# sikang/motion_primitive_library

Measured on NVIDIA H100. Metric: node-expansions/sec (frontier x |U| primitives validated+costed) on 512^3 voxel map, higher is better.
Workload: dtype f64

## Files before the change

### motion_primitive_library_b200/csrc/mplx_api.cu

```cuda
#include <cuda_runtime.h>
#include <math.h>
#include <stdarg.h>
#include <stdio.h>
#include <stdlib.h>
#include <string.h>

#include <new>
#include <vector>

#include "../../include/mplx.h"
#include "mplx_internal.h"
#include "mplx_pack.cuh"

namespace mplx {
thread_local char g_err[512] = "";
int fail(int code, const char *fmt, ...) {
  va_list ap;
  va_start(ap, fmt);
  vsnprintf(g_err, sizeof g_err, fmt, ap);
  va_end(ap);
  return code;
}
}
using mplx::g_err;

int mplx_bind(mplx_ctx *ctx) {
  if (!ctx) return fail(MPLX_ERR_ARG, "null ctx");
  CU(cudaSetDevice(ctx->device));
  return MPLX_OK;
}

static void refresh_params(mplx_ctx *c) {
  c->P.map = c->has_map ? c->map.p : nullptr;
  c->P.pot = c->has_pot ? c->pot.p : nullptr;
  c->P.region_bits = c->has_region ? c->region.p : nullptr;
  c->P.U = c->U.p;
  c->P.stats = c->stats_on ? c->stats.p : nullptr;
  c->P.occ_bits = c->has_map ? c->occ.p : nullptr;
  c->P.occ2 = c->has_map ? c->occ2.p : nullptr;
  c->P.occ2_bytes = c->has_map ? c->occ2_window : 0;
  c->P.prow = c->prow.p;
  c->P.row_u = c->row_u.p;
  c->P.row_axis = c->row_axis.p;
  c->P.n_rows = c->n_rows;
  c->P.ttab = c->ttab.p;
  c->P.tcount = c->tcount.p;
  c->P.tdt = c->tdt.p;
  int maxn = mplx::kNMax;
  if (c->has_map && c->has_params && (c->P.control & 15) != MPLX_VEL && c->P.v_max > 0) {
    const double nb = ceil(c->P.v_max * c->P.T / c->P.res);
    if (nb < (double)mplx::kNMax) maxn = nb < 5 ? 5 : (int)nb;
  }
  c->P.maxn = maxn;
}

extern "C" {

const char *mplx_last_error(void) { return g_err; }

const char *mplx_build_info(void) {
  return "libmplx sm_90a; nvcc -gencode arch=compute_90a,code=sm_90a -fmad=false; "
         "IEEE double, no CPU fallback";
}

int mplx_create(int dim, int device, mplx_ctx **out) {
  if (!out) return fail(MPLX_ERR_ARG, "out is null");
  *out = nullptr;
  if (dim != 2 && dim != 3) return fail(MPLX_ERR_ARG, "dim must be 2 or 3, got %d", dim);
  int ndev = 0;
  cudaError_t e = cudaGetDeviceCount(&ndev);
  if (e != cudaSuccess || ndev == 0) {
    cudaGetLastError();
    return fail(MPLX_ERR_CUDA, "no CUDA device available (%s); libmplx has no CPU fallback",
                e == cudaSuccess ? "device count is 0" : cudaGetErrorString(e));
  }
  if (device < 0 || device >= ndev) return fail(MPLX_ERR_ARG, "device %d out of range [0,%d)", device, ndev);
  CU(cudaSetDevice(device));
  mplx_ctx *c = new (std::nothrow) mplx_ctx();
  if (!c) return fail(MPLX_ERR_ALLOC, "host allocation failed");
  c->dim = dim;
  c->device = device;
  if (const char *k = getenv("MPLX_KERNEL")) {
    const int w = atoi(k);
    if (w >= 0 && w <= 5) c->kernel = w;
  }
  memset(&c->P, 0, sizeof c->P);
  c->P.dim = dim;
  e = cudaStreamCreateWithFlags(&c->stream, cudaStreamNonBlocking);
  if (e != cudaSuccess) {
    delete c;
    return fail(MPLX_ERR_CUDA, "cudaStreamCreate failed: %s", cudaGetErrorString(e));
  }
  e = c->stats.reserve(2);
  if (e != cudaSuccess) {
    cudaStreamDestroy(c->stream);
    delete c;
    return fail(MPLX_ERR_ALLOC, "cudaMalloc failed: %s", cudaGetErrorString(e));
  }
  *out = c;
  return MPLX_OK;
}

int mplx_destroy(mplx_ctx *c) {
  if (!c) return MPLX_OK;
  cudaSetDevice(c->device);
  cudaStreamSynchronize(c->stream);
  c->map.release(); c->pot.release(); c->region.release(); c->U.release(); c->stats.release();
  c->prow.release(); c->row_axis.release(); c->row_u.release();
  c->occ.release(); c->occ2.release(); c->ttab.release(); c->tcount.release(); c->tdt.release();
  for (int b = 0; b < kPackBufs; b++) c->cb[b].release();
  if (c->d2h_stream) cudaStreamDestroy(c->d2h_stream);
  c->eb.release(); c->fxq.release(); c->ub.release(); c->sb.release(); c->tun.release(); c->tb.release();
  c->d_nodes.release(); c->d_succ.release(); c->d_count.release(); c->d_action.release();
  c->d_lattice.release(); c->d_cost.release(); c->d_key.release();
  c->h_nodes.release(); c->h_succ.release(); c->h_count.release(); c->h_action.release();
  c->h_lattice.release(); c->h_cost.release(); c->h_key.release();
  cudaStreamDestroy(c->stream);
  delete c;
  return MPLX_OK;
}

int mplx_set_map(mplx_ctx *c, const int8_t *data, const int32_t *dim, const double *origin, double res) {
  if (int r = mplx_bind(c)) return r;
  if (!data || !dim || !origin) return fail(MPLX_ERR_ARG, "null argument");
  if (!(res > 0)) return fail(MPLX_ERR_ARG, "res must be > 0");
  size_t nvox = 1;
  for (int k = 0; k < c->dim; k++) {
    if (dim[k] <= 0) return fail(MPLX_ERR_ARG, "dim[%d] = %d", k, dim[k]);
    nvox *= (size_t)dim[k];
  }
  if (nvox >= (size_t)1 << 31) return fail(MPLX_ERR_ARG, "grid has %zu cells; getIndex is int32 (map_util.h:34-41)", nvox);
  CU(cudaStreamSynchronize(c->stream));
  CU(c->map.reserve(nvox));
  CU(cudaMemcpyAsync(c->map.p, data, nvox, cudaMemcpyHostToDevice, c->stream));
  CU(c->occ.reserve((nvox + 31) / 32));
  CU(mplx::launch_pack_bits(c->map.p, nvox, c->occ.p, true, c->stream));
  const int nz = c->dim == 3 ? dim[2] : 1;
  const size_t npairs = mplx::occ2_pair_count(c->dim, dim[0], dim[1], nz);
  CU(c->occ2.reserve(2 * npairs));
  CU(mplx::launch_pack_occ2(c->occ.p, nvox, c->dim, dim[0], dim[1], nz, c->occ2.p, c->stream));
  c->launches += 2;
  {
    int maxp = 0, maxw = 0;
    cudaDeviceGetAttribute(&maxp, cudaDevAttrMaxPersistingL2CacheSize, c->device);
    cudaDeviceGetAttribute(&maxw, cudaDevAttrMaxAccessPolicyWindowSize, c->device);
    const size_t half = npairs * sizeof(uint32_t);
    const size_t bytes = 2 * half <= (size_t)maxp ? 2 * half : half;
    c->occ2_window = 0;
    if (maxp > 0 && maxw > 0) {
      const size_t want = bytes < (size_t)maxp ? bytes : (size_t)maxp;
      if (cudaDeviceSetLimit(cudaLimitPersistingL2CacheSize, want) == cudaSuccess)
        c->occ2_window = bytes < (size_t)maxw ? bytes : (size_t)maxw;
      else
        cudaGetLastError();
    }
  }
  CU(cudaStreamSynchronize(c->stream));
  c->nvox = nvox;
  for (int k = 0; k < 3; k++) {
    c->P.mdim[k] = k < c->dim ? dim[k] : 1;
    c->P.origin[k] = k < c->dim ? origin[k] : 0.0;
    c->P.dimd[k] = (double)c->P.mdim[k];
  }
  c->P.occ2_nb[0] = mplx::occ2_bricks_x(c->dim, dim[0]);
  c->P.occ2_nb[1] = mplx::occ2_bricks_y(c->dim, dim[1]);
  c->P.occ2_sum = (unsigned)npairs;
  c->P.res = res;
  c->P.rinv = 1.0 / res;
  c->has_map = true;
  c->has_pot = false;
  c->has_region = false;
  c->tun.release();
  refresh_params(c);
  return MPLX_OK;
}

int mplx_set_potential(mplx_ctx *c, const int8_t *data, double pw, double gw) {
  if (int r = mplx_bind(c)) return r;
  if (!c->has_map) return fail(MPLX_ERR_ARG, "mplx_set_map must be called first");
  c->P.pot_w = pw;
  c->P.grad_w = gw;
  if (!data) {
    c->has_pot = false;
  } else {
    CU(cudaStreamSynchronize(c->stream));
    CU(c->pot.reserve(c->nvox));
    CU(cudaMemcpyAsync(c->pot.p, data, c->nvox, cudaMemcpyHostToDevice, c->stream));
    CU(cudaStreamSynchronize(c->stream));
    c->has_pot = true;
  }
  refresh_params(c);
  return MPLX_OK;
}

int mplx_set_potential_weights(mplx_ctx *c, double pw, double gw) {
  if (int r = mplx_bind(c)) return r;
  c->P.pot_w = pw;
  c->P.grad_w = gw;
  return MPLX_OK;
}

int mplx_set_search_region(mplx_ctx *c, const uint8_t *in_region) {
  if (int r = mplx_bind(c)) return r;
  if (!c->has_map) return fail(MPLX_ERR_ARG, "mplx_set_map must be called first");
  if (!in_region) {
    c->has_region = false;
  } else {
    CU(cudaStreamSynchronize(c->stream));
    DevBuf<uint8_t> tmp;
    CU(tmp.reserve(c->nvox));
    cudaError_t e = cudaMemcpyAsync(tmp.p, in_region, c->nvox, cudaMemcpyHostToDevice, c->stream);
    if (e == cudaSuccess) e = c->region.reserve((c->nvox + 31) / 32);
    if (e == cudaSuccess) e = mplx::launch_pack_bits((const int8_t *)tmp.p, c->nvox, c->region.p, false, c->stream);
    if (e == cudaSuccess) e = cudaStreamSynchronize(c->stream);
    tmp.release();
    CU(e);
    c->launches++;
    c->has_region = true;
  }
  refresh_params(c);
  return MPLX_OK;
}

int mplx_set_params(mplx_ctx *c, int control, double T, double w, double wyaw, double v_max,
                    double a_max, double j_max, double yaw_max, const double *U, int nU, int udim) {
  if (int r = mplx_bind(c)) return r;
  const int base = control & 15;
  if ((control & ~31) || (base != MPLX_VEL && base != MPLX_ACC && base != MPLX_JRK && base != MPLX_SNP))
    return fail(MPLX_ERR_ARG, "control 0x%x is not a Control::Control value (control.h:10-20)", control);
  const bool yaw = control & 16;
  if (!U || nU <= 0 || nU > mplx::kMaxU) return fail(MPLX_ERR_ARG, "need 1 <= nU <= %d controls", mplx::kMaxU);
  if (udim != c->dim + (yaw ? 1 : 0))
    return fail(MPLX_ERR_ARG, "udim %d must be dim%s = %d for control 0x%x", udim, yaw ? "+1" : "", c->dim + (yaw ? 1 : 0), control);
  if (!(T > 0)) return fail(MPLX_ERR_ARG, "T (dt_) must be > 0");
  CU(cudaStreamSynchronize(c->stream));
  CU(c->U.reserve((size_t)nU * udim));
  CU(cudaMemcpyAsync(c->U.p, U, sizeof(double) * nU * udim, cudaMemcpyHostToDevice, c->stream));
  {
    std::vector<unsigned char> prow((size_t)nU * 3, 0), row_axis;
    std::vector<double> row_u;
    bool fits = true;
    for (int a = 0; a < c->dim && fits; a++) {
      const size_t first = row_u.size();
      for (int i = 0; i < nU; i++) {
        const double v = U[(size_t)i * udim + a];
        size_t r = first;
        for (; r < row_u.size(); r++)
          if (memcmp(&row_u[r], &v, sizeof v) == 0) break;
        if (r == row_u.size()) {
          if (row_u.size() >= 255) { fits = false; break; }
          row_u.push_back(v);
          row_axis.push_back((unsigned char)a);
        }
        prow[(size_t)i * 3 + a] = (unsigned char)r;
      }
    }
    c->n_rows = 0;
    if (fits) {
      CU(c->prow.reserve(prow.size()));
      CU(c->row_u.reserve(row_u.size()));
      CU(c->row_axis.reserve(row_axis.size()));
      CU(cudaMemcpyAsync(c->prow.p, prow.data(), prow.size(), cudaMemcpyHostToDevice, c->stream));
      CU(cudaMemcpyAsync(c->row_u.p, row_u.data(), sizeof(double) * row_u.size(), cudaMemcpyHostToDevice, c->stream));
      CU(cudaMemcpyAsync(c->row_axis.p, row_axis.data(), row_axis.size(), cudaMemcpyHostToDevice, c->stream));
      CU(cudaStreamSynchronize(c->stream));
      c->n_rows = (int)row_u.size();
    }
  }
  CU(c->ttab.reserve((size_t)(mplx::kNMax + 1) * mplx::kTStride + 8));
  CU(c->tcount.reserve(mplx::kNMax + 1));
  CU(c->tdt.reserve(mplx::kNMax + 1));
  CU(cudaMemsetAsync(c->ttab.p, 0, sizeof(double) * ((size_t)(mplx::kNMax + 1) * mplx::kTStride + 8), c->stream));
  CU(mplx::launch_build_ttab(T, c->ttab.p, c->tcount.p, c->tdt.p, c->stream));
  c->launches++;
  CU(cudaStreamSynchronize(c->stream));
  c->P.control = control;
  c->P.nU = nU;
  c->P.udim = udim;
  c->P.T = T;
  c->P.w = w;
  c->P.wyaw = wyaw;
  c->P.v_max = v_max;
  c->P.a_max = a_max;
  c->P.j_max = j_max;
  c->P.yaw_max = yaw_max;
  c->P.cos_yaw_max = cos(yaw_max);
  c->has_params = true;
  refresh_params(c);
  return MPLX_OK;
}

int mplx_check_ready(mplx_ctx *c, int n_nodes) {
  if (!c->has_map) return fail(MPLX_ERR_ARG, "no map: call mplx_set_map first");
  if (!c->has_params) return fail(MPLX_ERR_ARG, "no params: call mplx_set_params first");
  if (n_nodes < 0) return fail(MPLX_ERR_ARG, "n_nodes < 0");
  if ((size_t)n_nodes * c->P.nU >= ((size_t)1 << 31)) return fail(MPLX_ERR_ARG, "batch too large");
  return MPLX_OK;
}
static int check_ready(mplx_ctx *c, int n_nodes, const mplx_succ_out *out) {
  if (int r = mplx_check_ready(c, n_nodes)) return r;
  if (!out || !out->count) return fail(MPLX_ERR_ARG, "out->count is required");
  return MPLX_OK;
}

int mplx_expand_device(mplx_ctx *c, const void *d_nodes, int n_nodes, const mplx_succ_out *out, void *stream) {
  if (int r = mplx_bind(c)) return r;
  if (int r = check_ready(c, n_nodes, out)) return r;
  if (n_nodes == 0) return MPLX_OK;
  if (!d_nodes) return fail(MPLX_ERR_ARG, "d_nodes is null");
  cudaStream_t st = stream ? (cudaStream_t)stream : c->stream;
  if (c->stats_on) CU(cudaMemsetAsync(c->stats.p, 0, 2 * sizeof(unsigned long long), st));
  CU(c->fxq.reserve((size_t)n_nodes * c->P.nU));
  int launches = 0;
  CU(mplx::launch_expand(c->P, (const mplx_waypoint *)d_nodes, n_nodes, *out, st, c->kernel, &c->fxq.view, &launches));
  c->launches += launches;
  if (c->stats_on)
    CU(cudaMemcpyAsync(c->last_stats, c->stats.p, 2 * sizeof(unsigned long long), cudaMemcpyDeviceToHost, st));
  return MPLX_OK;
}

int mplx_expand(mplx_ctx *c, const mplx_waypoint *nodes, int n_nodes, const mplx_succ_out *out) {
  if (int r = mplx_bind(c)) return r;
  if (int r = check_ready(c, n_nodes, out)) return r;
  if (n_nodes == 0) return MPLX_OK;
  if (!nodes) return fail(MPLX_ERR_ARG, "nodes is null");
  const int nU = c->P.nU;
  int chunk = (1 << 20) / nU;
  if (chunk < 1) chunk = 1;
  if (chunk > n_nodes) chunk = n_nodes;
  const size_t slots = (size_t)chunk * nU;
  cudaStream_t st = c->stream;

  CU(c->d_nodes.reserve(chunk));
  CU(c->d_count.reserve(chunk));
  if (out->succ) CU(c->d_succ.reserve(slots));
  if (out->cost) CU(c->d_cost.reserve(slots));
  if (out->action) CU(c->d_action.reserve(slots));
  if (out->key) CU(c->d_key.reserve(slots));
  if (out->lattice) CU(c->d_lattice.reserve(slots * MPLX_LATTICE_MAX));

  const bool pin_nodes = is_pinned(nodes), pin_count = is_pinned(out->count), pin_succ = is_pinned(out->succ),
             pin_cost = is_pinned(out->cost), pin_action = is_pinned(out->action), pin_key = is_pinned(out->key),
             pin_lat = is_pinned(out->lattice);
  if (!pin_nodes) CU(c->h_nodes.reserve(chunk));
  if (!pin_count) CU(c->h_count.reserve(chunk));
  if (out->succ && !pin_succ) CU(c->h_succ.reserve(slots));
  if (out->cost && !pin_cost) CU(c->h_cost.reserve(slots));
  if (out->action && !pin_action) CU(c->h_action.reserve(slots));
  if (out->key && !pin_key) CU(c->h_key.reserve(slots));
  if (out->lattice && !pin_lat) CU(c->h_lattice.reserve(slots * MPLX_LATTICE_MAX));

  static const bool no_zero_copy = getenv("MPLX_NO_ZERO_COPY") != nullptr;
  if (!no_zero_copy && !c->stats_on && (size_t)n_nodes * nU <= 4096) {
    const int m = n_nodes;
    const size_t sm = (size_t)m * nU;
    const mplx_waypoint *src = nodes;
    if (!pin_nodes) {
      memcpy(c->h_nodes.p, nodes, sizeof(mplx_waypoint) * m);
      src = c->h_nodes.p;
    }
    mplx_succ_out d;
    d.count = pin_count ? out->count : c->h_count.p;
    d.succ = out->succ ? (pin_succ ? out->succ : c->h_succ.p) : nullptr;
    d.cost = out->cost ? (pin_cost ? out->cost : c->h_cost.p) : nullptr;
    d.action = out->action ? (pin_action ? out->action : c->h_action.p) : nullptr;
    d.key = out->key ? (pin_key ? out->key : c->h_key.p) : nullptr;
    d.lattice = out->lattice ? (pin_lat ? out->lattice : c->h_lattice.p) : nullptr;
    CU(c->fxq.reserve(sm));
    int launches = 0;
    CU(mplx::launch_expand(c->P, src, m, d, st, c->kernel, &c->fxq.view, &launches));
    c->launches += launches;
    CU(cudaStreamSynchronize(st));
    if (!pin_count) memcpy(out->count, c->h_count.p, sizeof(int32_t) * m);
    if (out->succ && !pin_succ) memcpy(out->succ, c->h_succ.p, sizeof(mplx_waypoint) * sm);
    if (out->cost && !pin_cost) memcpy(out->cost, c->h_cost.p, sizeof(double) * sm);
    if (out->action && !pin_action) memcpy(out->action, c->h_action.p, sizeof(int32_t) * sm);
    if (out->key && !pin_key) memcpy(out->key, c->h_key.p, sizeof(uint64_t) * sm);
    if (out->lattice && !pin_lat) memcpy(out->lattice, c->h_lattice.p, sizeof(int32_t) * sm * MPLX_LATTICE_MAX);
    return MPLX_OK;
  }

  unsigned long long acc_stats[2] = {0, 0};
  for (int off = 0; off < n_nodes; off += chunk) {
    const int m = n_nodes - off < chunk ? n_nodes - off : chunk;
    const size_t so = (size_t)off * nU, sm = (size_t)m * nU;
    const mplx_waypoint *src = nodes + off;
    if (!pin_nodes) {
      memcpy(c->h_nodes.p, src, sizeof(mplx_waypoint) * m);
      src = c->h_nodes.p;
    }
    CU(cudaMemcpyAsync(c->d_nodes.p, src, sizeof(mplx_waypoint) * m, cudaMemcpyHostToDevice, st));
    mplx_succ_out d;
    d.count = c->d_count.p;
    d.succ = out->succ ? c->d_succ.p : nullptr;
    d.cost = out->cost ? c->d_cost.p : nullptr;
    d.action = out->action ? c->d_action.p : nullptr;
    d.key = out->key ? c->d_key.p : nullptr;
    d.lattice = out->lattice ? c->d_lattice.p : nullptr;
    if (c->stats_on) CU(cudaMemsetAsync(c->stats.p, 0, 2 * sizeof(unsigned long long), st));
    CU(c->fxq.reserve((size_t)m * nU));
    int launches = 0;
    CU(mplx::launch_expand(c->P, c->d_nodes.p, m, d, st, c->kernel, &c->fxq.view, &launches));
    c->launches += launches;
    if (c->stats_on)
      CU(cudaMemcpyAsync(c->last_stats, c->stats.p, 2 * sizeof(unsigned long long), cudaMemcpyDeviceToHost, st));
#define D2H(field, T, mult, pinflag, hbuf)                                                              \
  if (out->field) {                                                                                    \
    T *dst = pinflag ? out->field + so * (mult) : hbuf.p;                                              \
    CU(cudaMemcpyAsync(dst, d.field, sizeof(T) * sm * (mult), cudaMemcpyDeviceToHost, st));             \
  }
    {
      int32_t *dst = pin_count ? out->count + off : c->h_count.p;
      CU(cudaMemcpyAsync(dst, d.count, sizeof(int32_t) * m, cudaMemcpyDeviceToHost, st));
    }
    D2H(succ, mplx_waypoint, 1, pin_succ, c->h_succ)
    D2H(cost, double, 1, pin_cost, c->h_cost)
    D2H(action, int32_t, 1, pin_action, c->h_action)
    D2H(key, uint64_t, 1, pin_key, c->h_key)
    D2H(lattice, int32_t, MPLX_LATTICE_MAX, pin_lat, c->h_lattice)
#undef D2H
    CU(cudaStreamSynchronize(st));
    if (!pin_count) memcpy(out->count + off, c->h_count.p, sizeof(int32_t) * m);
    if (out->succ && !pin_succ) memcpy(out->succ + so, c->h_succ.p, sizeof(mplx_waypoint) * sm);
    if (out->cost && !pin_cost) memcpy(out->cost + so, c->h_cost.p, sizeof(double) * sm);
    if (out->action && !pin_action) memcpy(out->action + so, c->h_action.p, sizeof(int32_t) * sm);
    if (out->key && !pin_key) memcpy(out->key + so, c->h_key.p, sizeof(uint64_t) * sm);
    if (out->lattice && !pin_lat)
      memcpy(out->lattice + so * MPLX_LATTICE_MAX, c->h_lattice.p, sizeof(int32_t) * sm * MPLX_LATTICE_MAX);
    if (c->stats_on) {
      acc_stats[0] += c->last_stats[0];
      acc_stats[1] += c->last_stats[1];
    }
  }
  if (c->stats_on) {
    c->last_stats[0] = acc_stats[0];
    c->last_stats[1] = acc_stats[1];
  }
  return MPLX_OK;
}

int mplx_set_kernel(mplx_ctx *c, int which) {
  if (!c) return fail(MPLX_ERR_ARG, "null ctx");
  if (which < 0 || which > 5)
    return fail(MPLX_ERR_ARG, "which must be 0 (auto), 1 (sequential), 2 (register), 3 (flat), 4 (dealing) or 5 (fixed-point)");
  c->kernel = which;
  return MPLX_OK;
}

int mplx_sync(mplx_ctx *c) {
  if (int r = mplx_bind(c)) return r;
  CU(cudaStreamSynchronize(c->stream));
  return MPLX_OK;
}

int64_t mplx_launch_count(const mplx_ctx *c) { return c ? c->launches : 0; }

int mplx_enable_stats(mplx_ctx *c, int on) {
  if (int r = mplx_bind(c)) return r;
  c->stats_on = on != 0;
  refresh_params(c);
  return MPLX_OK;
}

int mplx_last_stats(mplx_ctx *c, int64_t *samples, int64_t *successors) {
  if (int r = mplx_bind(c)) return r;
  CU(cudaStreamSynchronize(c->stream));
  if (samples) *samples = (int64_t)c->last_stats[0];
  if (successors) *successors = (int64_t)c->last_stats[1];
  return MPLX_OK;
}

void *mplx_stream(mplx_ctx *c) { return c ? (void *)c->stream : nullptr; }

void *mplx_host_alloc(size_t bytes) {
  void *p = nullptr;
  if (cudaHostAlloc(&p, bytes, cudaHostAllocDefault) != cudaSuccess) {
    cudaGetLastError();
    fail(MPLX_ERR_ALLOC, "cudaHostAlloc(%zu) failed", bytes);
    return nullptr;
  }
  return p;
}

void mplx_host_free(void *p) {
  if (p) cudaFreeHost(p);
}

}
```

### motion_primitive_library_b200/csrc/mplx_device.cuh

```cuda
#pragma once
#include <limits.h>
#include <stdint.h>

namespace mplx {

struct EnvParams {
  int dim, control, nU, udim;
  double T, w, wyaw;
  double v_max, a_max, j_max, yaw_max;
  double cos_yaw_max;
  int mdim[3];
  double origin[3];
  double res;
  double rinv;
  double dimd[3];
  double pot_w, grad_w;
  const int8_t *map;
  const int8_t *pot;
  const uint32_t *region_bits;
  const double *U;
  unsigned long long *stats;
  const uint32_t *occ_bits;
  const double *ttab;
  const int *tcount;
  const double *tdt;
  int maxn;
  const uint32_t *occ2;
  unsigned occ2_sum;
  size_t occ2_bytes;
  int occ2_nb[2];
  const unsigned char *prow;
  const double *row_u;
  const unsigned char *row_axis;
  int n_rows;
};

constexpr int kNMax = 128;
constexpr int kTStride = kNMax + 2;

#define MPLX_PI 3.14159265358979323846

__device__ __forceinline__ double normalize_angle(double a) {
  while (a > MPLX_PI) a -= 2.0 * MPLX_PI;
  while (a < -MPLX_PI) a += 2.0 * MPLX_PI;
  return a;
}

__device__ __forceinline__ uint64_t hash_premix(int v) {
  uint64_t k = (uint64_t)(int64_t)v;
  const uint64_t m = 0xc6a4a7935bd1e995ULL;
  k *= m;
  k ^= k >> 47;
  k *= m;
  return k;
}
__device__ __forceinline__ void hash_fold(uint64_t &h, uint64_t k) {
  const uint64_t m = 0xc6a4a7935bd1e995ULL;
  h ^= k;
  h *= m;
  h += 0xe6546b64ULL;
}
__device__ __forceinline__ void hash_combine(uint64_t &h, int v) { hash_fold(h, hash_premix(v)); }

#define MPLX_MAGIC 6755399441055744.0

__device__ __forceinline__ double div_exact(double a, double b, double binv) {
  const double q0 = a * binv;
  const double r = __fma_rn(-b, q0, a);
  return __fma_rn(r, binv, q0);
}

__device__ __forceinline__ double round_haz(double x, int &k) {
  const double m = x + MPLX_MAGIC;
  double kd = m - MPLX_MAGIC;
  const double f = x - kd;
  k = __double2loint(m);
  if (fabs(f) == 0.5) {
    if (f > 0.0 && x > 0.0) { kd += 1.0; k += 1; }
    if (f < 0.0 && x < 0.0) { kd -= 1.0; k -= 1; }
  }
  return kd;
}

__device__ __forceinline__ int float_to_int(double p, double origin, double res) {
  const double x = (p - origin) / res - 0.5;
  if (!(fabs(x) < 2147483648.0)) return INT_MIN;
  int k;
  round_haz(x, k);
  return k;
}

__device__ __forceinline__ int lattice_id(double x, double res, double rinv) {
  int k;
  round_haz(div_exact(x, res, rinv), k);
  return k;
}

__device__ __forceinline__ double ceil_exact(double x) {
  const double kd = (x + MPLX_MAGIC) - MPLX_MAGIC;
  return kd < x ? kd + 1.0 : kd;
}

template <int ORD>
struct Axis {
  double c1, c2, c3, c4, c5;

  __device__ __forceinline__ void build(double u, double p, double v, double a, double j) {
    c1 = c2 = c3 = 0.0;
    if (ORD == 1) { c4 = u; c5 = p; }
    if (ORD == 2) { c3 = u; c4 = v; c5 = p; }
    if (ORD == 3) { c2 = u; c3 = a; c4 = v; c5 = p; }
    if (ORD == 4) { c1 = u; c2 = j; c3 = a; c4 = v; c5 = p; }
  }

  template <bool EXACT_ZERO>
  __device__ __forceinline__ double p(double t, double pw3, double pw4) const {
    if (EXACT_ZERO) {
      double s = 0.0;
      if (ORD >= 4) s = s + c1 / 24 * pw4;
      if (ORD >= 3) s = s + c2 / 6 * pw3;
      if (ORD >= 2) s = s + c3 / 2 * t * t;
      s = s + c4 * t;
      return s + c5;
    }
    if (ORD == 1) return c4 * t + c5;
    if (ORD == 2) return c3 / 2 * t * t + c4 * t + c5;
    if (ORD == 3) return c2 / 6 * pw3 + c3 / 2 * t * t + c4 * t + c5;
    return c1 / 24 * pw4 + c2 / 6 * pw3 + c3 / 2 * t * t + c4 * t + c5;
  }
  __device__ __forceinline__ double v(double t, double pw3) const {
    double s = 0.0;
    if (ORD >= 4) s = s + c1 / 6 * pw3;
    if (ORD >= 3) s = s + c2 / 2 * t * t;
    if (ORD >= 2) s = s + c3 * t;
    return s + c4;
  }
  __device__ __forceinline__ double a(double t) const {
    double s = 0.0;
    if (ORD >= 4) s = s + c1 / 2 * t * t;
    if (ORD >= 3) s = s + c2 * t;
    return s + c3;
  }
  __device__ __forceinline__ double j(double t) const {
    double s = 0.0;
    if (ORD >= 4) s = s + c1 * t;
    return s + c2;
  }

  __device__ __forceinline__ double max_vel(double T) const {
    double pw3T = (T * T) * T;
    double m = fmax(fabs(v(0.0, 0.0)), fabs(v(T, pw3T)));
    if (ORD >= 4 && c1 / 2 != 0) {
      double b = c1 / 2, c = c2, d = c3;
      double disc = c * c - 4 * b * d;
      if (!(disc < 0)) {
        double r0 = (-c - sqrt(disc)) / (2 * b);
        double r1 = (-c + sqrt(disc)) / (2 * b);
        bool brk = false;
        if (r0 > 0 && r0 < T) {
          double vv = fabs(v(r0, (r0 * r0) * r0));
          m = vv > m ? vv : m;
        } else if (r0 >= T)
          brk = true;
        if (!brk && r1 > 0 && r1 < T) {
          double vv = fabs(v(r1, (r1 * r1) * r1));
          m = vv > m ? vv : m;
        }
      }
    } else if (ORD >= 3 && c2 != 0) {
      double r = -c3 / c2;
      if (r > 0 && r < T) {
        double vv = fabs(v(r, (r * r) * r));
        m = vv > m ? vv : m;
      }
    }
    return m;
  }
  __device__ __forceinline__ double max_acc(double T) const {
    double m = fmax(fabs(a(0.0)), fabs(a(T)));
    if (ORD >= 4 && c1 != 0) {
      double r = -c2 / c1;
      if (r > 0 && r < T) {
        double aa = fabs(a(r));
        m = aa > m ? aa : m;
      }
    }
    return m;
  }
  __device__ __forceinline__ double max_jrk(double T) const { return fmax(fabs(j(0.0)), fabs(j(T))); }

  __device__ __forceinline__ double J(double T) const {
    double u = ORD == 1 ? c4 : ORD == 2 ? c3 : ORD == 3 ? c2 : c1;
    return u * u * T;
  }
};

__device__ __forceinline__ double dot2_normalized(double v0, double v1, double c, double s) {
  double z = v0 * v0 + v1 * v1;
  double n0 = v0, n1 = v1;
  if (z > 0) {
    double nn = sqrt(z);
    n0 = v0 / nn;
    n1 = v1 / nn;
  }
  return n0 * c + n1 * s;
}

}
```

### motion_primitive_library_b200/csrc/mplx_fx.cu

```cuda
#include "mplx_dispatch.h"
#include "mplx_fx.cuh"
#include "mplx_pack.cuh"

namespace mplx {

constexpr int kFxThreads = kThreads + 32;

struct FxShared {
  unsigned long long amask[kThreads];
  uint64_t hcurr[kThreads];
  double intrinsic[kThreads];
  unsigned slot[kThreads];
  uint32_t vbits[9];
  int q_n;
  unsigned char q[kThreads];
  unsigned char n[kThreads];
  unsigned char full[kThreads];
};

template <int DIM, int ORD, bool REGION>
__device__ __forceinline__ void fx_resolve(const EnvParams &P, const mplx_waypoint *__restrict__ nodes, int node0,
                                           int nU, int inv_nU, const FxShared &S, int lane, double *__restrict__ cost) {
  const int qn = S.q_n;
  for (int i = lane; i < qn; i += 32) {
    const int owner = S.q[i];
    const int nl = (owner * inv_nU) >> 20;
    const int ci = owner - nl * nU;
    const mplx_waypoint *cp = nodes + node0 + nl;
    const double *u = P.U + (size_t)ci * P.udim;
    PrimState<DIM, ORD, false> q;
#pragma unroll
    for (int k = 0; k < DIM; k++) q.ax[k].build(__ldg(u + k), cp->pos[k], cp->vel[k], cp->acc[k], cp->jrk[k]);
    double cf[CoefLayout<DIM, ORD, false>::NCMAX];
    fill_coef<DIM, ORD, false>(q, false, cf);
    const int n = S.n[owner];
    const double *tt = P.ttab + (size_t)n * kTStride;
    unsigned long long m = S.amask[owner];
    const int count = __ldg(P.tcount + n);
    const bool full = S.full[owner] != 0;
    bool blocked = false;
    for (int k = 0; !blocked; k++) {
      if (full) {
        if (k >= count) break;
      } else {
        if (m == 0) break;
        k = __ffsll((long long)m) - 1;
        m &= m - 1;
      }
      double pk[DIM];
      eval_pos<DIM, ORD>(cf, __ldg(tt + k), pk);
      int idx;
      blocked = !sample_cell<DIM>(P, pk, idx);
      if (!blocked) {
        blocked = (__ldg(P.occ_bits + (idx >> 5)) >> (idx & 31)) & 1u;
        if (REGION) blocked = blocked || !((__ldg(P.region_bits + (idx >> 5)) >> (idx & 31)) & 1u);
      }
    }
    if (cost) cost[S.slot[owner]] = blocked ? (double)INFINITY : 0.0 + S.intrinsic[owner];
  }
}

template <int DIM, int ORD, int UNR, int MINB, bool LAT, bool REGION>
__global__ void __launch_bounds__(kFxThreads, MINB)
expand_fx_kernel(const __grid_constant__ EnvParams P, const mplx_waypoint *__restrict__ nodes, int n_nodes, int npb,
                 int inv_nU, const __grid_constant__ OutPtrs o) {
  __shared__ FxShared S;
  const int nU = P.nU;
  const int items = npb * nU;
  const int node0 = blockIdx.x * npb;
  if (threadIdx.x >= kThreads) {
    const int lane = threadIdx.x - kThreads;
    if (lane == 0) S.q_n = 0;
    for (int j = lane; j < npb; j += 32)
      if (node0 + j < n_nodes) S.hcurr[j] = curr_hash<DIM, ORD>(nodes + node0 + j);
    __syncthreads();
    __syncthreads();
    __syncthreads();
    fx_resolve<DIM, ORD, REGION>(P, nodes, node0, nU, inv_nU, S, lane, o.cost);
    return;
  }

  const int item = threadIdx.x;
  const int nl = (item * inv_nU) >> 20;
  const int ci = item - nl * nU;
  const int ni = node0 + nl;
  const bool active = item < items && ni < n_nodes;
  PrimState<DIM, ORD, false> pr;
  bool ok = false, same = true;
  double max_v = 0;
  mplx_waypoint tn;
  int lat[LAT ? MPLX_LATTICE_MAX : 1];
  uint64_t key = 0;
  if (active) {
    const mplx_waypoint *cp = nodes + ni;
    const double *u = P.U + (size_t)ci * P.udim;
#pragma unroll
    for (int k = 0; k < DIM; k++) pr.ax[k].build(__ldg(u + k), cp->pos[k], cp->vel[k], cp->acc[k], cp->jrk[k]);
    const double T = P.T;
    const double pw3T = (T * T) * T, pw4T = pw3T * T;
#pragma unroll
    for (int k = 0; k < 3; k++) {
      if (k < DIM) {
        tn.pos[k] = pr.ax[k].template p<true>(T, pw3T, pw4T);
        tn.vel[k] = pr.ax[k].v(T, pw3T);
        tn.acc[k] = pr.ax[k].a(T);
        tn.jrk[k] = pr.ax[k].j(T);
        same = same && (pr.ax[k].c5 == tn.pos[k]);
      } else {
        tn.pos[k] = tn.vel[k] = tn.acc[k] = tn.jrk[k] = 0.0;
      }
    }
    tn.yaw = 0.0;
    tn.t = cp->t + T;
    ok = true;
#pragma unroll
    for (int k = 0; k < DIM; k++) {
      const double mv = pr.ax[k].max_vel(T);
      if (ORD >= 2 && P.v_max > 0) ok = ok && !(mv > P.v_max);
      if (mv > max_v) max_v = mv;
    }
    if (ok && ORD >= 3 && P.a_max > 0) {
#pragma unroll
      for (int k = 0; k < DIM; k++) ok = ok && !(pr.ax[k].max_acc(T) > P.a_max);
    }
    if (ok && ORD >= 4 && P.j_max > 0) {
#pragma unroll
      for (int k = 0; k < DIM; k++) ok = ok && !(pr.ax[k].max_jrk(T) > P.j_max);
    }
    if (ok) {
      int nl_ = 0;
#pragma unroll
      for (int k = 0; k < DIM; k++) {
        int id = lattice_id(tn.pos[k], 0.01, 100.0);
        hash_combine(key, id);
        if (LAT) lat[nl_++] = id;
        if (ORD >= 2) { id = lattice_id(tn.vel[k], 0.1, 10.0); hash_combine(key, id); if (LAT) lat[nl_++] = id; }
        if (ORD >= 3) { id = lattice_id(tn.acc[k], 0.1, 10.0); hash_combine(key, id); if (LAT) lat[nl_++] = id; }
        if (ORD >= 4) { id = lattice_id(tn.jrk[k], 0.1, 10.0); hash_combine(key, id); if (LAT) lat[nl_++] = id; }
      }
      if (LAT) {
#pragma unroll
        for (int q = 0; q < MPLX_LATTICE_MAX; q++)
          if (q >= nl_) lat[q] = 0;
      }
    }
  }
  __syncthreads();
  const bool emit = ok && key != S.hcurr[nl];

  const unsigned bal = __ballot_sync(0xffffffffu, emit);
  if ((threadIdx.x & 31) == 0) S.vbits[item >> 5] = bal;
  __syncthreads();
  size_t slot = 0;
  if (active) {
    const int s = nl * nU;
    int rank = 0;
    for (int wd = s >> 5; wd <= (item >> 5); wd++) {
      uint32_t m = S.vbits[wd];
      const int lo = wd << 5;
      if (s > lo) m &= ~0u << (s - lo);
      if (item < lo + 32) m &= (1u << (item - lo)) - 1u;
      rank += __popc(m);
    }
    if (ci == nU - 1) o.count[ni] = rank + (emit ? 1 : 0);
    if (emit) {
      slot = (size_t)ni * nU + rank;
      if (o.succ) store_waypoint(o.succ + slot, tn);
      if (o.action) __stcs(o.action + slot, ci);
      if (o.key) __stcs(reinterpret_cast<unsigned long long *>(o.key + slot), (unsigned long long)key);
      if (LAT && o.lattice) {
#pragma unroll
        for (int q = 0; q < MPLX_LATTICE_MAX; q++) o.lattice[slot * MPLX_LATTICE_MAX + q] = lat[q];
      }
    }
  }

  if (emit) {
    int verdict = 0;
    const double intrinsic = intrinsic_cost<DIM, ORD, false>(P, pr);
    if (!same) {
      double dt;
      const int n = sample_count_n(P, max_v, dt);
      double reach = 0.0;
#pragma unroll
      for (int a = 0; a < DIM; a++) reach = fmax(reach, (fabs(pr.ax[a].c5) + fabs(P.origin[a])) * P.rinv);
      if (n > kNMax || !(reach < kFxRange)) {
        double cf[CoefLayout<DIM, ORD, false>::NCMAX];
        fill_coef<DIM, ORD, false>(pr, false, cf);
        unsigned ns = 0;
        verdict = isinf(traverse_loop<DIM, ORD, false>(P, cf, false, max_v, ns)) ? 1 : 0;
      } else {
        double C[DIM][ORD + 1];
#pragma unroll
        for (int a = 0; a < DIM; a++) fx_axis<ORD>(pr.ax[a], P.origin[a], P.rinv, C[a]);
        const unsigned *__restrict__ occ_words = P.occ2;
        unsigned long long amask = 0;
        bool full = false;
        double t = 0;
        int base = 0;
        for (int left = __ldg(P.tcount + n);; left -= UNR, base += UNR) {
          unsigned amb;
          const int st = fx_group<DIM, ORD, UNR, REGION>(P, occ_words, C, dt, left, t, amb);
          if (st == 2) {
            verdict = 1;
            break;
          }
          if (amb) {
            if (base + UNR <= 64)
              amask |= (unsigned long long)amb << base;
            else
              full = true;
          }
          if (st == 1) break;
        }
        if (verdict == 0 && (amask != 0 || full)) {
          verdict = 2;
          const int qi = atomicAdd(&S.q_n, 1);
          S.q[qi] = (unsigned char)threadIdx.x;
          S.amask[threadIdx.x] = amask;
          S.n[threadIdx.x] = (unsigned char)n;
          S.full[threadIdx.x] = full ? 1 : 0;
          S.slot[threadIdx.x] = (unsigned)slot;
          S.intrinsic[threadIdx.x] = intrinsic;
        }
      }
    }
    if (verdict != 2 && o.cost) o.cost[slot] = verdict == 1 ? (double)INFINITY : 0.0 + intrinsic;
  }
  __syncthreads();
}

bool fx_supported(const EnvParams &P) {
  return P.occ2 != nullptr && P.pot == nullptr && (P.control & 16) == 0 && P.nU <= kThreads && P.stats == nullptr;
}

cudaError_t launch_expand_fx(const EnvParams &P, const mplx_waypoint *d_nodes, int n_nodes, const OutPtrs &o,
                             cudaStream_t st) {
  static const int unr_env = [] {
    const char *e = getenv("MPLX_FX_UNR");
    return e ? atoi(e) : 0;
  }();
  static const int minb_env = [] {
    const char *e = getenv("MPLX_FX_MINB");
    return e ? atoi(e) : 0;
  }();
  const int unr = unr_env == 4 || unr_env == 8 ? unr_env : (P.maxn <= 15 ? 4 : 8);
  const int npb = kThreads / P.nU;
  const int grid = (n_nodes + npb - 1) / npb;
  const int inv_nU = ((1 << 20) + P.nU - 1) / P.nU;
  return with_dim(P.dim, [&](auto DIM) {
    return with_order(P.control, [&](auto ORD) {
      return with_bool(unr == 8, [&](auto UNR8) {
        return with_bool(o.lattice != nullptr, [&](auto LAT) {
          return with_bool(P.region_bits != nullptr, [&](auto REGION) {
            auto launch = [&](auto MINB) {
              expand_fx_kernel<DIM, ORD, UNR8 ? 8 : 4, MINB, LAT, REGION>
                  <<<grid, kFxThreads, 0, st>>>(P, d_nodes, n_nodes, npb, inv_nU, o);
              return cudaGetLastError();
            };
            if constexpr (DIM == 3 && ORD == 2 && !LAT && !REGION) {
              if (minb_env == 5) return launch(Int<5>());
              if (minb_env == 6) return launch(Int<6>());
            }
            return launch(Int<4>());
          });
        });
      });
    });
  });
}

__global__ void pack_occ2_kernel(const uint32_t *__restrict__ occ, size_t nvox, int dim, int nx, int ny, int nz,
                                 uint32_t *__restrict__ out) {
  const size_t npairs = occ2_pair_count(dim, nx, ny, nz);
  for (size_t p = (size_t)blockIdx.x * blockDim.x + threadIdx.x; p < npairs; p += (size_t)gridDim.x * blockDim.x) {
    uint32_t o, s;
    occ2_brick_pair(occ, p, nvox, dim, nx, ny, nz, o, s);
    out[p] = o;
    out[npairs + p] = s;
  }
}

cudaError_t launch_pack_occ2(const uint32_t *d_occ, size_t nvox, int dim, int nx, int ny, int nz, uint32_t *d_out,
                             cudaStream_t st) {
  const size_t npairs = occ2_pair_count(dim, nx, ny, nz);
  int grid = (int)((npairs + 255) / 256);
  if (grid > sm_count() * 16) grid = sm_count() * 16;
  if (grid < 1) grid = 1;
  pack_occ2_kernel<<<grid, 256, 0, st>>>(d_occ, nvox, dim, nx, ny, nz, d_out);
  return cudaGetLastError();
}

}
```

### motion_primitive_library_b200/csrc/mplx_fx.cuh

```cuda
#pragma once
#include "mplx_expand.cuh"
#include "mplx_pack.cuh"

namespace mplx {

constexpr double kFxMagic = 1572864.0;
constexpr int kFxHiBase = 0x41380000;
constexpr double kFxEps = 0x1p-26;
constexpr unsigned kFxUnc = 128u;
constexpr double kFxRange = 131072.0;

template <int ORD>
__device__ __forceinline__ void fx_axis(const Axis<ORD> &ax, double origin, double rinv, double (&C)[ORD + 1]) {
  double q[5];
  q[0] = ax.c5;
  q[1] = ax.c4;
  q[2] = ax.c3 / 2;
  q[3] = ax.c2 / 6;
  q[4] = ax.c1 / 24;
#pragma unroll
  for (int i = 1; i <= ORD; i++) C[i] = q[i] * rinv;
  C[0] = (q[0] - origin) * rinv + (kFxMagic + kFxEps);
}

__device__ __forceinline__ unsigned rotr_wrap(unsigned x, unsigned s) {
  unsigned r;
  asm("shf.r.wrap.b32 %0, %1, %1, %2;" : "=r"(r) : "r"(x), "r"(s));
  return r;
}

template <int DIM, int ORD, int UNR, bool REGION>
__device__ __forceinline__ int fx_group(const EnvParams &P, const unsigned *__restrict__ base,
                                        const double (&C)[DIM][ORD + 1], double dt, int left, double &t, unsigned &amb) {
  unsigned w[UNR], rot[UNR];
  unsigned uncm = 0;
#pragma unroll
  for (int j = 0; j < UNR; j++) {
    int cell[DIM];
    unsigned lo[DIM];
    bool inside = true;
#pragma unroll
    for (int a = 0; a < DIM; a++) {
      double h = C[a][ORD];
#pragma unroll
      for (int i = ORD - 1; i >= 1; i--) h = __fma_rn(h, t, C[a][i]);
      const double m = __fma_rn(h, t, C[a][0]);
      cell[a] = __double2hiint(m) - kFxHiBase;
      lo[a] = (unsigned)__double2loint(m);
      inside = inside && ((unsigned)cell[a] < (unsigned)P.mdim[a]);
    }
    const unsigned fr = DIM == 3 ? min(min(lo[0], lo[1]), lo[DIM - 1]) : min(lo[0], lo[1]);
    const unsigned ub = fr < kFxUnc ? 1u : 0u;
    uncm += ub << j;
    w[j] = 0xffffffffu;
    if (REGION) {
      int idx = cell[0] + P.mdim[0] * cell[1];
      if (DIM == 3) idx += P.mdim[0] * P.mdim[1] * cell[DIM - 1];
      rot[j] = (unsigned)(idx - j);
      if (inside && !ub) {
        const unsigned wi = (unsigned)idx >> 5;
        w[j] = __ldg(P.occ_bits + wi) | ~__ldg(P.region_bits + wi);
      }
    } else {
      const int z = DIM == 3 ? cell[DIM - 1] : 0;
      rot[j] = occ2_bit<DIM>(cell[0], cell[1]) - j;
      if (inside) w[j] = __ldg(base + (occ2_pair<DIM>(cell[0], cell[1], z, P.occ2_nb[0], P.occ2_nb[1]) + (ub ? P.occ2_sum : 0u)));
    }
    t += dt;
  }
  unsigned r = 0;
#pragma unroll
  for (int j = 0; j < UNR; j++) r |= rotr_wrap(w[j], rot[j]) & (1u << j);
  if (left < UNR) r &= (1u << left) - 1u;
  amb = r & uncm;
  if (r & ~uncm) return 2;
  return left <= UNR ? 1 : 0;
}

template <int UNR>
struct FxWords {
  unsigned w[UNR], rot[UNR];
  unsigned uncm;
};

template <int DIM, int ORD, int UNR, bool REGION>
__device__ __forceinline__ void fx_issue(const EnvParams &P, const unsigned *__restrict__ base,
                                         const double (&C)[DIM][ORD + 1], double dt, double &t, FxWords<UNR> &G) {
  G.uncm = 0;
#pragma unroll
  for (int j = 0; j < UNR; j++) {
    int cell[DIM];
    unsigned lo[DIM];
    bool inside = true;
#pragma unroll
    for (int a = 0; a < DIM; a++) {
      double h = C[a][ORD];
#pragma unroll
      for (int i = ORD - 1; i >= 1; i--) h = __fma_rn(h, t, C[a][i]);
      const double m = __fma_rn(h, t, C[a][0]);
      cell[a] = __double2hiint(m) - kFxHiBase;
      lo[a] = (unsigned)__double2loint(m);
      inside = inside && ((unsigned)cell[a] < (unsigned)P.mdim[a]);
    }
    const unsigned fr = DIM == 3 ? min(min(lo[0], lo[1]), lo[DIM - 1]) : min(lo[0], lo[1]);
    const unsigned ub = fr < kFxUnc ? 1u : 0u;
    G.uncm += ub << j;
    G.w[j] = 0xffffffffu;
    if (REGION) {
      int idx = cell[0] + P.mdim[0] * cell[1];
      if (DIM == 3) idx += P.mdim[0] * P.mdim[1] * cell[DIM - 1];
      G.rot[j] = (unsigned)(idx - j);
      if (inside && !ub) {
        const unsigned wi = (unsigned)idx >> 5;
        G.w[j] = __ldg(P.occ_bits + wi) | ~__ldg(P.region_bits + wi);
      }
    } else {
      const int z = DIM == 3 ? cell[DIM - 1] : 0;
      G.rot[j] = occ2_bit<DIM>(cell[0], cell[1]) - j;
      if (inside) G.w[j] = __ldg(base + (occ2_pair<DIM>(cell[0], cell[1], z, P.occ2_nb[0], P.occ2_nb[1]) + (ub ? P.occ2_sum : 0u)));
    }
    t += dt;
  }
}

template <int UNR>
__device__ __forceinline__ int fx_decide(const FxWords<UNR> &G, int left, unsigned &amb) {
  unsigned r = 0;
#pragma unroll
  for (int j = 0; j < UNR; j++) r |= rotr_wrap(G.w[j], G.rot[j]) & (1u << j);
  if (left < UNR) r &= (1u << left) - 1u;
  amb = r & G.uncm;
  if (r & ~G.uncm) return 2;
  return left <= UNR ? 1 : 0;
}

template <int DIM, int ORD, int UNR, bool REGION>
__device__ __forceinline__ int fx_traverse(const EnvParams &P, const double (&C)[DIM][ORD + 1], double dt, int count,
                                           unsigned long long &amask, bool &full) {
  const unsigned *__restrict__ base = P.occ2;
  amask = 0;
  full = false;
  double t = 0;
  int left = count, k0 = 0;
  FxWords<UNR> A, B;
  fx_issue<DIM, ORD, UNR, REGION>(P, base, C, dt, t, A);
  for (;;) {
    unsigned amb;
    int st;
    if (left > UNR) fx_issue<DIM, ORD, UNR, REGION>(P, base, C, dt, t, B);
    st = fx_decide<UNR>(A, left, amb);
    if (st == 2) return 1;
    if (amb) {
      if (k0 + UNR <= 64) amask |= (unsigned long long)amb << k0; else full = true;
    }
    if (st == 1) return 0;
    left -= UNR;
    k0 += UNR;
    if (left > UNR) fx_issue<DIM, ORD, UNR, REGION>(P, base, C, dt, t, A);
    st = fx_decide<UNR>(B, left, amb);
    if (st == 2) return 1;
    if (amb) {
      if (k0 + UNR <= 64) amask |= (unsigned long long)amb << k0; else full = true;
    }
    if (st == 1) return 0;
    left -= UNR;
    k0 += UNR;
  }
}

template <int DIM, int ORD>
__device__ __forceinline__ uint64_t curr_hash(const mplx_waypoint *cp) {
  uint64_t h = 0;
#pragma unroll
  for (int k = 0; k < DIM; k++) {
    hash_combine(h, lattice_id(cp->pos[k], 0.01, 100.0));
    if (ORD >= 2) hash_combine(h, lattice_id(cp->vel[k], 0.1, 10.0));
    if (ORD >= 3) hash_combine(h, lattice_id(cp->acc[k], 0.1, 10.0));
    if (ORD >= 4) hash_combine(h, lattice_id(cp->jrk[k], 0.1, 10.0));
  }
  return h;
}

constexpr unsigned kFxSegments = 64;

struct FxAmbRec {
  unsigned slot;
  int node;
  unsigned short action;
  unsigned char n;
  unsigned char full;
  unsigned long long amask;
};

}
```

### motion_primitive_library_b200/csrc/mplx_fxn.cu

```cuda
#include <string.h>

#include "mplx_dispatch.h"
#include "mplx_fx.cuh"
#include "mplx_span.cuh"

namespace mplx {

template <int ORD>
struct FxnRow {
  double st[4];
  double C[ORD + 1];
  double mv;
  double J;
  int id[4];
  uint64_t km[ORD];
  unsigned char f0, f1, f2, pad[5];
};
constexpr unsigned char kSame = 1, kReach = 2, kVel = 1, kAcc = 1, kJrk = 2;


struct FxnWork {
  unsigned rows_n;
  unsigned slot;
};

constexpr int kMaxNpb = kThreads / 9;
struct FxnShared {
  uint64_t hcurr[kMaxNpb];
  uint64_t ckm[kMaxNpb * 3 * 4];
  double tcurr[kMaxNpb];
  FxnWork work[kThreads];
  unsigned char owner[kThreads];
  uint32_t vbits[8];
  unsigned short cnt[kWarps][33], start[kWarps][33];
};
constexpr unsigned kNoWork = 0xffffffffu;

struct FxnStage {
  int succ, key, action, cost;
};
constexpr int kSpanUnsorted = 7, kSpanMinLoop = 20;

__device__ __forceinline__ void bulk_copy(void *g, const unsigned char *s, unsigned bytes) {
  const unsigned sa = (unsigned)__cvta_generic_to_shared(s);
  asm volatile("cp.async.bulk.global.shared::cta.bulk_group [%0], [%1], %2;" ::"l"(g), "r"(sa), "r"(bytes) : "memory");
}

__device__ __forceinline__ void span_out(void *g, const unsigned char *s, unsigned elem, unsigned n) {
  const SpanCopy c = span_copy(reinterpret_cast<uintptr_t>(g), elem, n);
  unsigned char *d = static_cast<unsigned char *>(g);
  const unsigned end = elem * n, trail0 = end - c.trail;
  for (unsigned i = 0; i < c.lead; i += 4) *reinterpret_cast<uint32_t *>(d + i) = *reinterpret_cast<const uint32_t *>(s + i);
  for (unsigned i = trail0; i < end; i += 4) *reinterpret_cast<uint32_t *>(d + i) = *reinterpret_cast<const uint32_t *>(s + i);
  unsigned at = c.lead;
  if (c.head) bulk_copy(d + at, s + at, c.head);
  at += c.head;
  if (c.body) bulk_copy(d + at, s + at, c.body);
  at += c.body;
  if (c.tail) bulk_copy(d + at, s + at, c.tail);
}

template <int DIM, int ORD, int UNR, int MINB, bool LAT, bool REGION, bool SORT, bool STAGE>
__global__ void __launch_bounds__(kThreads, MINB)
expand_fxn_kernel(const __grid_constant__ EnvParams P, const mplx_waypoint *__restrict__ nodes, int n_nodes, int npb,
                  int inv_nU, int inv_rows, FxAmbRec *__restrict__ amb_q, unsigned *__restrict__ amb_n,
                  unsigned amb_cap, const __grid_constant__ OutPtrs o, int pf_ahead, const FxnStage sg) {
  extern __shared__ __align__(16) unsigned char fx_dyn[];
  FxnRow<ORD> *rows = reinterpret_cast<FxnRow<ORD> *>(fx_dyn);
  __shared__ FxnShared S;
  const int nU = P.nU;
  const int items = npb * nU;
  const int node0 = blockIdx.x * npb;
  const int n_rows = P.n_rows;
  const int lane = threadIdx.x & 31, warp = threadIdx.x >> 5;

  if (SORT) {
    for (int b = threadIdx.x; b < kWarps * 33; b += kThreads) (&S.cnt[0][0])[b] = 0;
    S.work[threadIdx.x].slot = kNoWork;
  }
  if (pf_ahead > 0 && threadIdx.x < 16) {
    const long long first = ((long long)blockIdx.x + pf_ahead) * npb;
    const char *pfp = reinterpret_cast<const char *>(nodes + first) + 128 * threadIdx.x;
    if (first < n_nodes && pfp < reinterpret_cast<const char *>(nodes + min((long long)n_nodes, first + npb)))
      asm volatile("prefetch.global.L2 [%0];" ::"l"(pfp));
  }

  {
    const double T = P.T;
    const int R = npb * n_rows;
    const int tail = (3 * R) & (kThreads - 1);
    const bool hash_warp = warp == (tail <= kThreads - 32 ? kWarps - 1 : tail >> 5);
    double cx[2] = {0.0, 0.0}, ct = 0.0;
    auto load_ids = [&] {
      constexpr int F = DIM * ORD;
#pragma unroll
      for (int k = 0; k < 2; k++) {
        const int q = lane + 32 * k;
        const int j = q / F, af = q - j * F;
        if (q < npb * F && node0 + j < n_nodes)
          cx[k] = reinterpret_cast<const double *>(nodes + node0 + j)[(af % ORD) * 3 + af / ORD];
      }
      if (lane < npb && node0 + lane < n_nodes) ct = nodes[node0 + lane].t;
    };
    if (hash_warp) load_ids();
    for (int it = threadIdx.x; it < 3 * R; it += kThreads) {
      const int part = it >= 2 * R ? 2 : (it >= R ? 1 : 0);
      const int r = it - part * R;
      const int nl = (r * inv_rows) >> 20;
      const int rr = r - nl * n_rows;
      if (node0 + nl >= n_nodes) continue;
      const mplx_waypoint *cp = nodes + node0 + nl;
      const int a = __ldg(P.row_axis + rr);
      Axis<ORD> ax;
      ax.build(__ldg(P.row_u + rr), cp->pos[a], cp->vel[a], cp->acc[a], cp->jrk[a]);
      FxnRow<ORD> &Rw = rows[r];
      if (part == 0) {
        const double origin = a == 0 ? P.origin[0] : (a == 1 ? P.origin[1] : P.origin[2]);
        const double pw3T = (T * T) * T, pw4T = pw3T * T;
        const double pos = ax.template p<true>(T, pw3T, pw4T);
        Rw.st[0] = pos;
        const int id = lattice_id(pos, 0.01, 100.0);
        Rw.id[0] = id;
        Rw.km[0] = hash_premix(id);
        unsigned char f = 0;
        if (ax.c5 == pos) f |= kSame;
        if ((fabs(ax.c5) + fabs(origin)) * P.rinv < kFxRange) f |= kReach;
        Rw.f0 = f;
        Rw.J = ax.J(T);
      } else if (part == 1) {
        const double pw3T = (T * T) * T;
        const double vel = ax.v(T, pw3T);
        Rw.st[1] = vel;
        const int id = ORD >= 2 ? lattice_id(vel, 0.1, 10.0) : 0;
        Rw.id[1] = id;
        if (ORD >= 2) Rw.km[ORD >= 2 ? 1 : 0] = hash_premix(id);
        const double mv = ax.max_vel(T);
        Rw.mv = mv;
        Rw.f1 = (ORD >= 2 && P.v_max > 0 && mv > P.v_max) ? 0 : kVel;
      } else {
        const double origin = a == 0 ? P.origin[0] : (a == 1 ? P.origin[1] : P.origin[2]);
        fx_axis<ORD>(ax, origin, P.rinv, Rw.C);
        const double acc = ax.a(T), jrk = ax.j(T);
        Rw.st[2] = acc;
        Rw.st[3] = jrk;
        Rw.id[2] = ORD >= 3 ? lattice_id(acc, 0.1, 10.0) : 0;
        Rw.id[3] = ORD >= 4 ? lattice_id(jrk, 0.1, 10.0) : 0;
        if (ORD >= 3) Rw.km[ORD >= 3 ? 2 : 0] = hash_premix(Rw.id[2]);
        if (ORD >= 4) Rw.km[ORD >= 4 ? 3 : 0] = hash_premix(Rw.id[3]);
        unsigned char f = kAcc | kJrk;
        if (ORD >= 3 && P.a_max > 0 && ax.max_acc(T) > P.a_max) f &= ~kAcc;
        if (ORD >= 4 && P.j_max > 0 && ax.max_jrk(T) > P.j_max) f &= ~kJrk;
        Rw.f2 = f;
      }
    }
    if (hash_warp) {
      constexpr int F = DIM * ORD;
#pragma unroll
      for (int k = 0; k < 2; k++) {
        const int q = lane + 32 * k;
        if (q < npb * F) {
          const bool is_pos = (q % F) % ORD == 0;
          S.ckm[q] = hash_premix(lattice_id(cx[k], is_pos ? 0.01 : 0.1, is_pos ? 100.0 : 10.0));
        }
      }
      for (int q = lane + 64; q < npb * F; q += 32) {
        const int j = q / F, af = q - j * F;
        const bool is_pos = af % ORD == 0;
        const double x = node0 + j < n_nodes ? reinterpret_cast<const double *>(nodes + node0 + j)[(af % ORD) * 3 + af / ORD] : 0.0;
        S.ckm[q] = hash_premix(lattice_id(x, is_pos ? 0.01 : 0.1, is_pos ? 100.0 : 10.0));
      }
      __syncwarp();
      for (int j = lane; j < npb; j += 32) {
        uint64_t h = 0;
#pragma unroll
        for (int af = 0; af < F; af++) hash_fold(h, S.ckm[j * F + af]);
        S.hcurr[j] = h;
        if (j == lane) S.tcurr[j] = ct;
        else if (node0 + j < n_nodes) S.tcurr[j] = nodes[node0 + j].t;
      }
    }
  }
  __syncthreads();

  const int item = threadIdx.x;
  const int nl = (item * inv_nU) >> 20;
  const int ci = item - nl * nU;
  const int ni = node0 + nl;
  const bool active = item < items && ni < n_nodes;
  bool ok = false, same = true, reach = true;
  double max_v = 0;
  uint64_t key = 0;
  int ra[DIM];
#pragma unroll
  for (int a = 0; a < DIM; a++) ra[a] = 0;
  if (active) {
    unsigned f0 = kSame | kReach, f1 = kVel, f2 = kAcc | kJrk;
#pragma unroll
    for (int a = 0; a < DIM; a++) {
      ra[a] = nl * n_rows + __ldg(P.prow + ci * 3 + a);
      const FxnRow<ORD> &Rw = rows[ra[a]];
      f0 &= Rw.f0;
      f1 &= Rw.f1;
      f2 &= Rw.f2;
      if (Rw.mv > max_v) max_v = Rw.mv;
    }
    ok = f1 == kVel && f2 == (kAcc | kJrk);
    same = (f0 & kSame) != 0;
    reach = (f0 & kReach) != 0;
    if (ok) {
#pragma unroll
      for (int a = 0; a < DIM; a++) {
        const FxnRow<ORD> &Rw = rows[ra[a]];
#pragma unroll
        for (int f = 0; f < ORD; f++) hash_fold(key, Rw.km[f]);
      }
    }
  }
  const bool emit = ok && key != S.hcurr[nl];

  int n = 0, count = 0;
  double dt = 0.0;
  const bool literal = emit && !same && !reach;
  bool beyond = false;
  if (emit && !same) {
    n = sample_count_n(P, max_v, dt);
    beyond = n > kNMax;
    if (!beyond && !literal) count = __ldg(P.tcount + n);
  }
  const int g = (count + UNR - 1) / UNR;
  const int gk = g > 32 ? 32 : g;
  int bin_rank = 0;
  if (SORT) {
    const unsigned peers = __match_any_sync(0xffffffffu, gk);
    bin_rank = __popc(peers & ((1u << lane) - 1u));
    if (gk > 0 && bin_rank == 0) S.cnt[warp][gk] = (unsigned short)__popc(peers);
  }

  const unsigned bal = __ballot_sync(0xffffffffu, emit);
  if (lane == 0) S.vbits[warp] = bal;
  __syncthreads();
  if (SORT) {
    if (warp == 0) {
      unsigned c[kWarps], tot = 0;
#pragma unroll
      for (int w = 0; w < kWarps; w++) {
        c[w] = S.cnt[w][lane + 1];
        tot += c[w];
      }
      unsigned above = tot;
#pragma unroll
      for (int d = 1; d < 32; d <<= 1) {
        const unsigned v = __shfl_down_sync(0xffffffffu, above, d);
        if (lane + d < 32) above += v;
      }
      unsigned at = above - tot;
#pragma unroll
      for (int w = 0; w < kWarps; w++) {
        S.start[w][lane + 1] = (unsigned short)at;
        at += c[w];
      }
    }
    __syncthreads();
  }
  static_assert(!(SORT && STAGE), "the sorted path writes its outputs per lane");
  const size_t span0 = (size_t)node0 * nU;
  const unsigned span_n = (unsigned)((n_nodes - node0 < npb ? n_nodes - node0 : npb) * nU);
  auto staged = [&](int off, const void *gptr) { return fx_dyn + off + (reinterpret_cast<uintptr_t>(gptr) & 15u); };
  size_t slot = 0;
  double intrinsic = 0.0;
  if (active) {
    const int s = nl * nU;
    int rank = 0;
    if (nU <= 32) {
      const unsigned below = (1u << lane) - 1u;
      if ((s >> 5) == warp) {
        rank = __popc(bal & below & (~0u << (s & 31)));
      } else {
        rank = __popc(bal & below) + __popc(S.vbits[warp - 1] >> (s & 31));
      }
    } else {
      for (int wd = s >> 5; wd <= (item >> 5); wd++) {
        uint32_t m = S.vbits[wd];
        const int lo = wd << 5;
        if (s > lo) m &= ~0u << (s - lo);
        if (item < lo + 32) m &= (1u << (item - lo)) - 1u;
        rank += __popc(m);
      }
    }
    if (ci == nU - 1) o.count[ni] = rank + (emit ? 1 : 0);
    if constexpr (STAGE) {
      const int sl = s + (emit ? rank : nU - 1 - (ci - rank));
      mplx_waypoint tn = {};
      if (emit) {
#pragma unroll
        for (int k = 0; k < DIM; k++) {
          const FxnRow<ORD> &Rw = rows[ra[k]];
          tn.pos[k] = Rw.st[0];
          tn.vel[k] = Rw.st[1];
          tn.acc[k] = Rw.st[2];
          tn.jrk[k] = Rw.st[3];
        }
        tn.t = S.tcurr[nl] + P.T;
      }
      double2 *sp = reinterpret_cast<double2 *>(fx_dyn + sg.succ + sl * (int)sizeof(mplx_waypoint));
      sp[0] = make_double2(tn.pos[0], tn.pos[1]);
      sp[1] = make_double2(tn.pos[2], tn.vel[0]);
      sp[2] = make_double2(tn.vel[1], tn.vel[2]);
      sp[3] = make_double2(tn.acc[0], tn.acc[1]);
      sp[4] = make_double2(tn.acc[2], tn.jrk[0]);
      sp[5] = make_double2(tn.jrk[1], tn.jrk[2]);
      sp[6] = make_double2(tn.yaw, tn.t);
      if (sg.key >= 0) reinterpret_cast<uint64_t *>(staged(sg.key, o.key + span0))[sl] = emit ? key : 0;
      if (sg.action >= 0) reinterpret_cast<int32_t *>(staged(sg.action, o.action + span0))[sl] = emit ? ci : 0;
      if (sg.cost >= 0 && !emit) reinterpret_cast<double *>(staged(sg.cost, o.cost + span0))[sl] = 0.0;
    } else if (o.succ && emit) {
      mplx_waypoint tn;
#pragma unroll
      for (int k = 0; k < 3; k++) {
        if (k < DIM) {
          const FxnRow<ORD> &Rw = rows[ra[k < DIM ? k : 0]];
          tn.pos[k] = Rw.st[0];
          tn.vel[k] = Rw.st[1];
          tn.acc[k] = Rw.st[2];
          tn.jrk[k] = Rw.st[3];
        } else {
          tn.pos[k] = tn.vel[k] = tn.acc[k] = tn.jrk[k] = 0.0;
        }
      }
      tn.yaw = 0.0;
      tn.t = S.tcurr[nl] + P.T;
      store_waypoint(o.succ + (size_t)ni * nU + rank, tn);
    }
    if (emit) {
      slot = (size_t)ni * nU + rank;
      if (o.action && !(STAGE && sg.action >= 0)) __stcs(o.action + slot, ci);
      if (o.key && !(STAGE && sg.key >= 0))
        __stcs(reinterpret_cast<unsigned long long *>(o.key + slot), (unsigned long long)key);
      if (LAT && o.lattice) {
        int q = 0;
#pragma unroll
        for (int a = 0; a < DIM; a++) {
          const FxnRow<ORD> &Rw = rows[ra[a]];
#pragma unroll
          for (int f = 0; f < ORD; f++) o.lattice[slot * MPLX_LATTICE_MAX + q++] = Rw.id[f];
        }
        for (; q < MPLX_LATTICE_MAX; q++) o.lattice[slot * MPLX_LATTICE_MAX + q] = 0;
      }
      double J = rows[ra[0]].J;
#pragma unroll
      for (int a = 1; a < DIM; a++) J += rows[ra[a]].J;
      intrinsic = J + P.w * P.T;
    }
  }

  FxnWork wk;
  wk.rows_n = (unsigned)ra[0] | ((unsigned)ra[1] << 8) | ((unsigned)(DIM == 3 ? ra[DIM - 1] : 0) << 16) | ((unsigned)n << 24);
  wk.slot = g > 0 ? (unsigned)slot : kNoWork;
  int wowner = threadIdx.x;
  if (SORT && g > 0) {
    const int pos = (int)S.start[warp][gk] + bin_rank;
    S.work[pos] = wk;
    S.owner[pos] = (unsigned char)threadIdx.x;
  }
  if (emit && g == 0) {
    int v = 0;
    if (literal || beyond) {
      PrimState<DIM, ORD, false> pr;
      const mplx_waypoint *cp = nodes + ni;
      const double *u = P.U + (size_t)ci * P.udim;
#pragma unroll
      for (int k = 0; k < DIM; k++) pr.ax[k].build(__ldg(u + k), cp->pos[k], cp->vel[k], cp->acc[k], cp->jrk[k]);
      double cf[CoefLayout<DIM, ORD, false>::NCMAX];
      fill_coef<DIM, ORD, false>(pr, false, cf);
      unsigned ns = 0;
      v = isinf(traverse_loop<DIM, ORD, false>(P, cf, false, max_v, ns)) ? 1 : 0;
    }
    const double c = v == 1 ? (double)INFINITY : 0.0 + intrinsic;
    if (STAGE && sg.cost >= 0) reinterpret_cast<double *>(staged(sg.cost, o.cost + span0))[slot - span0] = c;
    else if (o.cost) o.cost[slot] = c;
  }
  if (SORT) {
    __syncthreads();
    wk = S.work[threadIdx.x];
    wowner = S.owner[threadIdx.x];
  }

  bool bulk_issued = false;
  if constexpr (STAGE) {
    asm volatile("fence.proxy.async.shared::cta;" ::: "memory");
    __syncthreads();
    if (threadIdx.x == 0) {
      span_out(o.succ + span0, fx_dyn + sg.succ, (unsigned)sizeof(mplx_waypoint), span_n);
      if (sg.key >= 0) span_out(o.key + span0, staged(sg.key, o.key + span0), 8u, span_n);
      if (sg.action >= 0) span_out(o.action + span0, staged(sg.action, o.action + span0), 4u, span_n);
      asm volatile("cp.async.bulk.commit_group;" ::: "memory");
      bulk_issued = true;
    }
  }

  int verdict = -1;
  unsigned long long amask = 0;
  bool full = false;
  unsigned wslot = 0;
  int wn = 0;
  double wintr = 0.0;
  if (wk.slot != kNoWork) {
    wslot = wk.slot;
    wn = (int)(wk.rows_n >> 24);
    int wr[DIM];
    wr[0] = wk.rows_n & 255u;
    wr[1] = (wk.rows_n >> 8) & 255u;
    if (DIM == 3) wr[DIM - 1] = (wk.rows_n >> 16) & 255u;
    double C[DIM][ORD + 1];
#pragma unroll
    for (int a = 0; a < DIM; a++) {
      const FxnRow<ORD> &Rw = rows[wr[a]];
#pragma unroll
      for (int i = 0; i <= ORD; i++) C[a][i] = Rw.C[i];
    }
    double J = rows[wr[0]].J;
#pragma unroll
    for (int a = 1; a < DIM; a++) J += rows[wr[a]].J;
    wintr = J + P.w * P.T;
    verdict = fx_traverse<DIM, ORD, UNR, REGION>(P, C, __ldg(P.tdt + wn), __ldg(P.tcount + wn), amask, full);
    if (verdict == 0 && (amask != 0 || full)) verdict = 2;
  }
  const unsigned am = __ballot_sync(0xffffffffu, verdict == 2);
  if (am) {
    const unsigned seg = blockIdx.x & (kFxSegments - 1);
    const unsigned segcap = amb_cap / kFxSegments;
    unsigned base = 0;
    const int leader = __ffs(am) - 1;
    if (lane == leader) base = atomicAdd(amb_n + seg, (unsigned)__popc(am));
    base = __shfl_sync(0xffffffffu, base, leader);
    if (verdict == 2) {
      const unsigned pos = base + __popc(am & ((1u << lane) - 1u));
      if (pos < segcap) {
        FxAmbRec rec;
        const int onl = (wowner * inv_nU) >> 20;
        rec.slot = wslot;
        rec.node = node0 + onl;
        rec.action = (unsigned short)(wowner - onl * nU);
        rec.n = (unsigned char)wn;
        rec.full = full ? 1 : 0;
        rec.amask = amask;
        amb_q[(size_t)seg * segcap + pos] = rec;
      } else {
        verdict = 3;
      }
    }
  }
  if (verdict == 3) {
    const int onl = (wowner * inv_nU) >> 20;
    PrimState<DIM, ORD, false> pr;
    const mplx_waypoint *cp = nodes + node0 + onl;
    const double *u = P.U + (size_t)(wowner - onl * nU) * P.udim;
    double mv = 0;
#pragma unroll
    for (int k = 0; k < DIM; k++) {
      pr.ax[k].build(__ldg(u + k), cp->pos[k], cp->vel[k], cp->acc[k], cp->jrk[k]);
      const double m1 = pr.ax[k].max_vel(P.T);
      if (m1 > mv) mv = m1;
    }
    double cf[CoefLayout<DIM, ORD, false>::NCMAX];
    fill_coef<DIM, ORD, false>(pr, false, cf);
    unsigned ns = 0;
    verdict = isinf(traverse_loop<DIM, ORD, false>(P, cf, false, mv, ns)) ? 1 : 0;
  }
  if (STAGE && sg.cost >= 0) {
    if (verdict >= 0)
      reinterpret_cast<double *>(staged(sg.cost, o.cost + span0))[wslot - (unsigned)span0] =
          verdict == 1 ? (double)INFINITY : (verdict == 2 ? 0.0 : 0.0 + wintr);
    asm volatile("fence.proxy.async.shared::cta;" ::: "memory");
    __syncthreads();
    if (threadIdx.x == 0) {
      span_out(o.cost + span0, staged(sg.cost, o.cost + span0), 8u, span_n);
      asm volatile("cp.async.bulk.commit_group;" ::: "memory");
      bulk_issued = true;
    }
  } else if ((verdict == 0 || verdict == 1) && o.cost) {
    __stcs(o.cost + wslot, verdict == 1 ? (double)INFINITY : 0.0 + wintr);
  }
  if (bulk_issued) asm volatile("cp.async.bulk.wait_group.read 0;" ::: "memory");
}

template <int DIM, int ORD, bool REGION>
__global__ void __launch_bounds__(128)
fx_resolve_kernel(const __grid_constant__ EnvParams P, const mplx_waypoint *__restrict__ nodes,
                  const FxAmbRec *__restrict__ amb_q, const unsigned *__restrict__ amb_n, unsigned amb_cap,
                  double *__restrict__ cost) {
  const unsigned seg = blockIdx.x & (kFxSegments - 1);
  const unsigned segcap = amb_cap / kFxSegments;
  unsigned total = amb_n[seg];
  if (total > segcap) total = segcap;
  const unsigned sib = blockIdx.x / kFxSegments, nsib = gridDim.x / kFxSegments;
  for (unsigned i = sib * blockDim.x + threadIdx.x; i < total; i += nsib * blockDim.x) {
    const FxAmbRec rec = amb_q[(size_t)seg * segcap + i];
    const mplx_waypoint *cp = nodes + rec.node;
    const double *u = P.U + (size_t)rec.action * P.udim;
    PrimState<DIM, ORD, false> pr;
#pragma unroll
    for (int k = 0; k < DIM; k++) pr.ax[k].build(__ldg(u + k), cp->pos[k], cp->vel[k], cp->acc[k], cp->jrk[k]);
    double cf[CoefLayout<DIM, ORD, false>::NCMAX];
    fill_coef<DIM, ORD, false>(pr, false, cf);
    const int n = rec.n;
    const double *tt = P.ttab + (size_t)n * kTStride;
    unsigned long long m = rec.amask;
    const int count = __ldg(P.tcount + n);
    const bool full = rec.full != 0;
    bool blocked = false;
    for (int k = 0; !blocked; k++) {
      if (full) {
        if (k >= count) break;
      } else {
        if (m == 0) break;
        k = __ffsll((long long)m) - 1;
        m &= m - 1;
      }
      double pk[DIM];
      eval_pos<DIM, ORD>(cf, __ldg(tt + k), pk);
      int idx;
      blocked = !sample_cell<DIM>(P, pk, idx);
      if (!blocked) {
        blocked = (__ldg(P.occ_bits + (idx >> 5)) >> (idx & 31)) & 1u;
        if (REGION) blocked = blocked || !((__ldg(P.region_bits + (idx >> 5)) >> (idx & 31)) & 1u);
      }
    }
    if (cost) cost[rec.slot] = blocked ? (double)INFINITY : 0.0 + intrinsic_cost<DIM, ORD, false>(P, pr);
  }
}

bool fxn_supported(const EnvParams &P, int n_nodes) {
  if (!fx_supported(P) || P.n_rows <= 0 || P.nU > kThreads) return false;
  if (P.n_rows * 2 > P.dim * P.nU) return false;
  const int npb = kThreads / P.nU;
  if (npb * P.n_rows > 255 || npb > kMaxNpb) return false;
  const size_t smem = (size_t)npb * P.n_rows * 128;
  if (smem > 64 * 1024) return false;
  return (long)n_nodes * P.nU >= 64L * kThreads;
}

cudaError_t launch_expand_fxn(const EnvParams &P, const mplx_waypoint *d_nodes, int n_nodes, const OutPtrs &o,
                              cudaStream_t st, void *amb_q, unsigned *amb_n, unsigned amb_cap) {
  FxAmbRec *q = static_cast<FxAmbRec *>(amb_q);
  const int npb = kThreads / P.nU;
  const int grid = (n_nodes + npb - 1) / npb;
  const bool lat = o.lattice != nullptr;
  const bool region = P.region_bits != nullptr;
  const int inv_nU = ((1 << 20) + P.nU - 1) / P.nU;
  const int inv_rows = ((1 << 20) + P.n_rows - 1) / P.n_rows;
  static const int sort_env = [] { const char *v = getenv("MPLX_FXN_SORT"); return v ? atoi(v) : -1; }();
  static const int span_env = [] { const char *v = getenv("MPLX_FXN_SPAN"); return v ? atoi(v) : -1; }();
  cudaError_t e = cudaMemsetAsync(amb_n, 0, sizeof(unsigned) * kFxSegments, st);
  if (e != cudaSuccess) return e;
  static const bool no_window = getenv("MPLX_NO_L2_WINDOW") != nullptr;
  if (!no_window && P.occ2_bytes > 0) {
    cudaStreamAttrValue av;
    memset(&av, 0, sizeof av);
    av.accessPolicyWindow.base_ptr = const_cast<uint32_t *>(P.occ2);
    av.accessPolicyWindow.num_bytes = P.occ2_bytes;
    av.accessPolicyWindow.hitRatio = 1.0f;
    av.accessPolicyWindow.hitProp = cudaAccessPropertyPersisting;
    av.accessPolicyWindow.missProp = cudaAccessPropertyStreaming;
    if (cudaStreamSetAttribute(st, cudaStreamAttributeAccessPolicyWindow, &av) != cudaSuccess) cudaGetLastError();
  }
  static const int carve = [] { const char *v = getenv("MPLX_FXN_CARVE"); return v ? atoi(v) : -1; }();
  static const int pf_env = [] { const char *v = getenv("MPLX_FXN_PREFETCH"); return v ? atoi(v) : -1; }();
  const int pf_ahead = pf_env >= 0 ? pf_env : 2 * 4 * sm_count();
  static const int unr_env = [] { const char *v = getenv("MPLX_FXN_UNR"); return v ? atoi(v) : 0; }();
  static const int minb_env = [] { const char *v = getenv("MPLX_FXN_MINB"); return v ? atoi(v) : 0; }();
  return with_dim(P.dim, [&](auto DIM) {
    return with_order(P.control, [&](auto ORD) {
      const int rows_bytes = (int)(((size_t)npb * P.n_rows * sizeof(FxnRow<ORD>) + 15) & ~(size_t)15);
      const bool sort = sort_env >= 0 ? sort_env != 0 : ORD >= 3;
      const int mask = sort ? 0 : span_env >= 0 ? span_env : P.maxn >= kSpanMinLoop ? kSpanUnsorted : 1;
      const size_t span_slots = (size_t)npb * P.nU;
      FxnStage sg = {-1, -1, -1, -1};
      size_t smem = (size_t)rows_bytes;
      auto take = [&](size_t bytes) {
        const int off = (int)smem;
        smem += (bytes + 16 + 15) & ~(size_t)15;
        return off;
      };
      if ((mask & 1) && o.succ && (reinterpret_cast<uintptr_t>(o.succ) & 15u) == 0)
        sg.succ = take(span_slots * sizeof(mplx_waypoint));
      constexpr size_t kCtaSmem = 48 * 1024;
      const size_t ka = (o.key ? span_slots * 8 + 32 : 0) + (o.action ? span_slots * 4 + 32 : 0);
      if ((mask & 2) && sg.succ >= 0 && ka > 0 && smem + ka + sizeof(FxnShared) <= kCtaSmem) {
        if (o.key) sg.key = take(span_slots * 8);
        if (o.action) sg.action = take(span_slots * 4);
      }
      if ((mask & 4) && sg.succ >= 0 && o.cost && smem + span_slots * 8 + 32 + sizeof(FxnShared) <= kCtaSmem)
        sg.cost = take(span_slots * 8);
      auto launch = [&](auto UNR, auto MINB, auto LAT, auto REGION) {
        auto go = [&](auto SORT, auto STAGE) {
          const auto kernel = expand_fxn_kernel<DIM, ORD, UNR, MINB, LAT, REGION, SORT, STAGE>;
          if (smem > 32 * 1024) {
            const cudaError_t r = cudaFuncSetAttribute(kernel, cudaFuncAttributeMaxDynamicSharedMemorySize, (int)smem);
            if (r != cudaSuccess) return r;
          }
          if (carve >= 0) {
            const cudaError_t r = cudaFuncSetAttribute(kernel, cudaFuncAttributePreferredSharedMemoryCarveout, carve);
            if (r != cudaSuccess) return r;
          }
          kernel<<<grid, kThreads, smem, st>>>(P, d_nodes, n_nodes, npb, inv_nU, inv_rows, q, amb_n, amb_cap, o,
                                                pf_ahead, sg);
          return cudaGetLastError();
        };
        if (sort) return go(std::true_type{}, std::false_type{});
        return with_bool(sg.succ >= 0, [&](auto STAGE) { return go(std::false_type{}, STAGE); });
      };
      const std::true_type yes{};
      const std::false_type no{};
      if (region) e = with_bool(lat, [&](auto LAT) { return launch(Int<4>(), Int<4>(), LAT, yes); });
      else if (lat) e = launch(Int<4>(), Int<4>(), yes, no);
      else if (unr_env == 8 && minb_env == 3) e = launch(Int<8>(), Int<3>(), no, no);
      else if (unr_env == 4 && minb_env == 3) e = launch(Int<4>(), Int<3>(), no, no);
      else if (unr_env == 8) e = launch(Int<8>(), Int<4>(), no, no);
      else if (minb_env == 5) e = launch(Int<4>(), Int<5>(), no, no);
      else e = launch(Int<4>(), Int<4>(), no, no);
      if (e != cudaSuccess) return e;
      return with_bool(region, [&](auto REGION) {
        fx_resolve_kernel<DIM, ORD, REGION><<<kFxSegments * 8, 128, 0, st>>>(P, d_nodes, q, amb_n, amb_cap, o.cost);
        return cudaGetLastError();
      });
    });
  });
}

size_t fx_amb_record_bytes() { return sizeof(FxAmbRec); }

}
```

### motion_primitive_library_b200/csrc/mplx_internal.h

```cpp
#pragma once
#include <cuda_runtime.h>
#include <stdarg.h>
#include <stdint.h>
#include <stdio.h>

#include <vector>
#include "../../include/mplx.h"
#include "mplx_device.cuh"
#include "mplx_kernels.h"

namespace mplx {
int fail(int code, const char *fmt, ...);
}
using mplx::fail;

#define CU(call)                                                                              \
  do {                                                                                        \
    cudaError_t e_ = (call);                                                                  \
    if (e_ != cudaSuccess) {                                                                  \
      cudaGetLastError();                                                                     \
      return fail(e_ == cudaErrorMemoryAllocation ? MPLX_ERR_ALLOC : MPLX_ERR_CUDA,           \
                  "%s failed: %s (%s:%d)", #call, cudaGetErrorString(e_), __FILE__, __LINE__); \
    }                                                                                         \
  } while (0)

template <typename T>
struct DevBuf {
  T *p = nullptr;
  size_t cap = 0;
  cudaError_t reserve(size_t n) {
    if (n <= cap) return cudaSuccess;
    if (p) cudaFree(p);
    p = nullptr;
    cap = 0;
    cudaError_t e = cudaMalloc((void **)&p, n * sizeof(T));
    if (e == cudaSuccess) cap = n;
    return e;
  }
  void release() {
    if (p) cudaFree(p);
    p = nullptr;
    cap = 0;
  }
};

template <typename T>
struct ScopedDevBuf : DevBuf<T> {
  ScopedDevBuf() = default;
  ScopedDevBuf(const ScopedDevBuf &) = delete;
  ScopedDevBuf &operator=(const ScopedDevBuf &) = delete;
  ~ScopedDevBuf() { this->release(); }
};

struct TimedRun {
  cudaEvent_t e0 = nullptr, e1 = nullptr;
  TimedRun() = default;
  TimedRun(const TimedRun &) = delete;
  TimedRun &operator=(const TimedRun &) = delete;
  ~TimedRun() {
    if (e0) cudaEventDestroy(e0);
    if (e1) cudaEventDestroy(e1);
  }
  template <class F>
  cudaError_t run(cudaStream_t st, int64_t &launches, F &&launch) {
    cudaError_t e = cudaEventCreate(&e0);
    if (e == cudaSuccess) e = cudaEventCreate(&e1);
    if (e != cudaSuccess) return e;
    int n = 0;
    e = cudaEventRecord(e0, st);
    if (e == cudaSuccess) e = launch(&n);
    if (e == cudaSuccess) e = cudaEventRecord(e1, st);
    launches += n;
    return e;
  }
  cudaError_t seconds(double *s) const {
    float ms = 0.f;
    const cudaError_t e = cudaEventElapsedTime(&ms, e0, e1);
    *s = ms * 1e-3;
    return e;
  }
};

template <typename T>
struct PinBuf {
  T *p = nullptr;
  size_t cap = 0;
  cudaError_t reserve(size_t n) {
    if (n <= cap) return cudaSuccess;
    if (p) cudaFreeHost(p);
    p = nullptr;
    cap = 0;
    cudaError_t e = cudaHostAlloc((void **)&p, n * sizeof(T), cudaHostAllocDefault);
    if (e == cudaSuccess) cap = n;
    return e;
  }
  void release() {
    if (p) cudaFreeHost(p);
    p = nullptr;
    cap = 0;
  }
};

inline bool is_pinned(const void *p) {
  if (!p) return false;
  cudaPointerAttributes a;
  if (cudaPointerGetAttributes(&a, p) != cudaSuccess) {
    cudaGetLastError();
    return false;
  }
  return a.type == cudaMemoryTypeHost;
}

struct FxQueue {
  DevBuf<unsigned char> q;
  DevBuf<unsigned> n;
  mplx::FxScratch view;
  cudaError_t reserve(size_t n_prims) {
    const size_t cap = ((n_prims / 4 + 64 * 4096 + 63) / 64) * 64;
    cudaError_t e = q.reserve(cap * mplx::fx_amb_record_bytes());
    if (e == cudaSuccess) e = n.reserve(64);
    if (e != cudaSuccess) return e;
    view.q = q.p;
    view.n = n.p;
    view.cap = (unsigned)(q.cap / mplx::fx_amb_record_bytes() / 64 * 64);
    return cudaSuccess;
  }
  void release() { q.release(); n.release(); view = mplx::FxScratch(); }
};

constexpr int kPackBufs = 4;
struct ChunkBufs {
  cudaStream_t st = nullptr;
  cudaEvent_t ready = nullptr;
  cudaEvent_t drained = nullptr;
  DevBuf<mplx_waypoint> nodes, succ;
  DevBuf<int32_t> count, action;
  DevBuf<double> cost;
  DevBuf<uint64_t> key;
  DevBuf<int32_t> kcount;
  DevBuf<long long> offset, total;
  DevBuf<double> pstate, pcost;
  DevBuf<uint16_t> paction;
  DevBuf<uint64_t> pkey;
  PinBuf<long long> h_total;
  FxQueue fxq;
  void release() {
    fxq.release();
    nodes.release(); succ.release(); count.release(); action.release(); cost.release(); key.release();
    kcount.release(); offset.release(); total.release(); pstate.release(); pcost.release(); paction.release();
    pkey.release(); h_total.release();
    if (ready) cudaEventDestroy(ready);
    if (drained) cudaEventDestroy(drained);
    if (st) cudaStreamDestroy(st);
    ready = drained = nullptr;
    st = nullptr;
  }
};

struct EdgeBufs {
  DevBuf<mplx_waypoint> parents;
  DevBuf<int32_t> actions, cells, ids, owner, ids_sorted, owner_sorted;
  DevBuf<uint8_t> free_, scan_tmp;
  DevBuf<double> cost;
  DevBuf<long long> count, offset;
  void release() {
    parents.release(); actions.release(); cells.release(); free_.release(); scan_tmp.release(); cost.release();
    count.release(); offset.release(); ids.release(); owner.release(); ids_sorted.release(); owner_sorted.release();
  }
};

struct UpdateBufs {
  PinBuf<uint32_t> h_idx;
  PinBuf<int8_t> h_val;
  DevBuf<uint32_t> idx, idx_sorted;
  DevBuf<int8_t> val, val_sorted;
  DevBuf<uint8_t> sort_tmp;
  void release() {
    h_idx.release(); h_val.release(); idx.release(); idx_sorted.release(); val.release(); val_sorted.release();
    sort_tmp.release();
  }
};

struct TrajBufs {
  DevBuf<long long> offset;
  DevBuf<mplx_waypoint> wps;
  DevBuf<uint8_t> ctl, mono;
  DevBuf<int32_t> status;
  DevBuf<double> dts, seg_t, taus, coeff, samples, fac, dpos, dyaw;
  DevBuf<int32_t> n_cand, n_knot;
  DevBuf<double> par, total, seg_T, cand, cand_p, knot_t, knot_p, lam, lam_T;
  DevBuf<int32_t> n_pts;
  DevBuf<uint8_t> form, seg_free, seg_valid;
  DevBuf<double> cost;
  DevBuf<long long> slot_src;
  DevBuf<int32_t> slot_action;
  void release() {
    slot_src.release(); slot_action.release();
    offset.release(); wps.release(); ctl.release(); mono.release(); status.release(); dts.release(); seg_t.release();
    taus.release(); coeff.release(); samples.release(); fac.release(); dpos.release(); dyaw.release();
    n_cand.release(); n_knot.release(); par.release(); total.release(); seg_T.release(); cand.release();
    cand_p.release(); knot_t.release(); knot_p.release(); lam.release(); lam_T.release();
    n_pts.release(); form.release(); seg_free.release(); seg_valid.release(); cost.release();
  }
};

constexpr size_t kSearchArenaBudget = (size_t)8 << 30;

enum TrajState : int { kTrajNone = 0, kTrajOff = 1, kTrajOn = 2 };
struct SearchBufs {
  DevBuf<unsigned char> arena;
  int64_t layout_bytes = 0;
  size_t cleared = 0;
  uint32_t next_epoch = 1;
  DevBuf<mplx_waypoint> succ, queries;
  DevBuf<double> cost, dres;
  DevBuf<uint64_t> key, closed;
  DevBuf<int32_t> action, count, ires;
  DevBuf<uint8_t> free_;
  DevBuf<unsigned long long> offs;
  std::vector<int64_t> grow_aoff, grow_coff;
  std::vector<int32_t> grow_actions;
  std::vector<uint64_t> grow_closed;
  bool traj_on = false;
  int64_t traj_room_bytes = 0;
  DevBuf<mplx_waypoint> traj;
  int64_t traj_kept = 0;
  DevBuf<unsigned long long> toffs;
  int traj_state = 0;
  std::vector<int64_t> traj_off, slot_src;
  std::vector<int32_t> slot_action;
  void release() {
    arena.release(); succ.release(); queries.release(); cost.release(); dres.release(); key.release();
    closed.release(); action.release(); count.release(); ires.release(); free_.release(); offs.release();
    traj.release(); toffs.release();
    traj_kept = 0;
    traj_state = 0;
    layout_bytes = 0;
    cleared = 0;
    next_epoch = 1;
  }
};

struct TunnelStore {
  int n_q = 0;
  int64_t n_bricks = 0;
  DevBuf<uint64_t> key;
  DevBuf<uint32_t> bits;
  DevBuf<int64_t> off;
  size_t bytes() const { return key.cap * sizeof(uint64_t) + bits.cap * sizeof(uint32_t) + off.cap * sizeof(int64_t); }
  void release() {
    key.release(); bits.release(); off.release();
    n_q = 0;
    n_bricks = 0;
  }
};

struct mplx_ctx {
  int dim = 0, device = 0;
  cudaStream_t stream = nullptr;
  DevBuf<int8_t> map, pot;
  DevBuf<uint32_t> region, occ;
  DevBuf<uint32_t> occ2;
  DevBuf<unsigned char> prow, row_axis;
  DevBuf<double> row_u;
  int n_rows = 0;
  size_t occ2_window = 0;
  DevBuf<double> U, ttab, tdt;
  DevBuf<int> tcount;
  int kernel = 0;
  DevBuf<unsigned long long> stats;
  bool has_map = false, has_pot = false, has_region = false, has_params = false, stats_on = false;
  size_t nvox = 0;
  mplx::EnvParams P;
  DevBuf<mplx_waypoint> d_nodes, d_succ;
  DevBuf<int32_t> d_count, d_action, d_lattice;
  DevBuf<double> d_cost;
  DevBuf<uint64_t> d_key;
  PinBuf<mplx_waypoint> h_nodes, h_succ;
  PinBuf<int32_t> h_count, h_action, h_lattice;
  PinBuf<double> h_cost;
  PinBuf<uint64_t> h_key;
  ChunkBufs cb[kPackBufs];
  cudaStream_t d2h_stream = nullptr;
  FxQueue fxq;
  EdgeBufs eb;
  UpdateBufs ub;
  SearchBufs sb;
  TunnelStore tun;
  TrajBufs tb;
  int64_t launches = 0;
  unsigned long long last_stats[2] = {0, 0};
};

namespace mplx {
namespace search {
struct Grid;
}
search::Grid region_grid(const mplx_ctx *c);
void region_radius_cells(const mplx_ctx *c, const double *radius, int *rn);
int search_budget(const mplx_ctx *c, size_t &budget);
}

extern "C" {
int mplx_bind(mplx_ctx *ctx);
int mplx_check_ready(mplx_ctx *c, int n_nodes);
}
```

### motion_primitive_library_b200/csrc/mplx_maps.cu

```cuda
#include <cuda_runtime.h>
#include <math.h>
#include <string.h>

#include <algorithm>
#include <vector>

#include "mplx_internal.h"
#include "mplx_search.cuh"

namespace mplx {

constexpr int kNoRank = 255;

__global__ void source_bits_kernel(const int8_t *__restrict__ map, int nx, int ny, int nz, int lo0, int lo1, int lo2,
                                   int hi0, int hi1, int hi2, uint32_t *__restrict__ bits) {
  const size_t nvox = (size_t)nx * ny * nz;
  const size_t nwords = (nvox + 31) >> 5;
  for (size_t wd = (size_t)blockIdx.x * blockDim.x + threadIdx.x; wd < nwords; wd += (size_t)gridDim.x * blockDim.x) {
    uint32_t m = 0;
    for (int b = 0; b < 32; b++) {
      const size_t i = (wd << 5) + b;
      if (i >= nvox) break;
      const int x = (int)(i % nx), y = (int)((i / nx) % ny), z = (int)(i / ((size_t)nx * ny));
      if (map[i] > 0 && x >= lo0 && x < hi0 && y >= lo1 && y < hi1 && z >= lo2 && z < hi2) m |= 1u << b;
    }
    bits[wd] = m;
  }
}

__global__ void layer_rank_kernel(const uint32_t *__restrict__ src, int nx, int ny, int nz, int rn,
                                  const uint8_t *__restrict__ pair_rank, uint8_t *__restrict__ rank) {
  const size_t nvox = (size_t)nx * ny * nz;
  for (size_t i = (size_t)blockIdx.x * blockDim.x + threadIdx.x; i < nvox; i += (size_t)gridDim.x * blockDim.x) {
    const int x = (int)(i % nx), y = (int)((i / nx) % ny), z = (int)(i / ((size_t)nx * ny));
    int best = kNoRank;
    const int x0 = max(0, x - rn), x1 = min(nx - 1, x + rn);
    for (int yy = max(0, y - rn); yy <= min(ny - 1, y + rn); yy++) {
      const size_t row = ((size_t)z * ny + yy) * nx;
      const uint8_t *pr = pair_rank + (size_t)abs(yy - y) * (rn + 1);
      const size_t b0 = row + x0, b1 = row + x1;
      for (size_t wd = b0 >> 5; wd <= (b1 >> 5); wd++) {
        uint32_t m = __ldg(src + wd);
        const size_t base = wd << 5;
        if (base < b0) m &= ~0u << (b0 - base);
        if (base + 31 > b1) m &= ~0u >> (base + 31 - b1);
        while (m) {
          const int b = __ffs(m) - 1;
          m &= m - 1;
          const int xx = (int)(base + b - row);
          best = min(best, (int)pr[abs(xx - x)]);
        }
      }
    }
    rank[i] = (uint8_t)best;
  }
}

__global__ void potential_combine_kernel(const int8_t *__restrict__ map, const uint32_t *__restrict__ src,
                                         const uint8_t *__restrict__ rank, int nx, int ny, int nz, int hn,
                                         const int8_t *__restrict__ htab, int8_t *__restrict__ out) {
  const size_t nvox = (size_t)nx * ny * nz, layer = (size_t)nx * ny;
  for (size_t i = (size_t)blockIdx.x * blockDim.x + threadIdx.x; i < nvox; i += (size_t)gridDim.x * blockDim.x) {
    const int z = (int)(i / layer);
    int v = map[i];
    if ((src[i >> 5] >> (i & 31)) & 1u) v = 100;
    for (int dz = -hn; dz <= hn; dz++) {
      const int zs = z - dz;
      if (zs < 0 || zs >= nz) continue;
      const int r = rank[i - (size_t)dz * layer];
      if (r != kNoRank) v = max(v, (int)htab[r * (hn + 1) + abs(dz)]);
    }
    out[i] = (int8_t)v;
  }
}

__global__ void region_stamp_kernel(const int *__restrict__ cells, int n_cells, int dim, int nx, int ny, int nz, int r0,
                                    int r1, int r2, uint32_t *__restrict__ bits) {
  const int w0 = 2 * r0 + 1, w1 = 2 * r1 + 1, w2 = dim == 3 ? 2 * r2 + 1 : 1;
  const size_t per = (size_t)w0 * w1 * w2, total = per * n_cells;
  for (size_t t = (size_t)blockIdx.x * blockDim.x + threadIdx.x; t < total; t += (size_t)gridDim.x * blockDim.x) {
    const int c = (int)(t / per);
    size_t o = t % per;
    const int dx = (int)(o % w0) - r0;
    o /= w0;
    const int dy = (int)(o % w1) - r1;
    o /= w1;
    const int dz = dim == 3 ? (int)o - r2 : 0;
    const int x = cells[c * 3] + dx, y = cells[c * 3 + 1] + dy, z = cells[c * 3 + 2] + dz;
    if (x < 0 || x >= nx || y < 0 || y >= ny || z < 0 || z >= nz) continue;
    const size_t idx = (size_t)x + (size_t)nx * y + (size_t)nx * ny * z;
    atomicOr(bits + (idx >> 5), 1u << (idx & 31));
  }
}

static int grid_for(size_t n) {
  size_t g = (n + 255) / 256;
  const size_t cap = (size_t)sm_count() * 32;
  if (g > cap) g = cap;
  return g < 1 ? 1 : (int)g;
}

}

using namespace mplx;

static void float_to_int(const mplx_ctx *c, const double *pt, int *pn) {
  for (int k = 0; k < 3; k++) pn[k] = k < c->dim ? (int)std::round((pt[k] - c->P.origin[k]) / c->P.res - 0.5) : 0;
}

extern "C" int mplx_update_potential_map(mplx_ctx *c, const double *radius, double pow_, const double *range,
                                         const double *pos, double potential_weight, double gradient_weight,
                                         int8_t *out_map) {
  if (int r = mplx_bind(c)) return r;
  if (!c->has_map) return fail(MPLX_ERR_ARG, "mplx_set_map must be called first");
  if (!radius) return fail(MPLX_ERR_ARG, "radius is null");
  if (!(pow_ > 0)) return fail(MPLX_ERR_ARG, "pow must be > 0 (the stencil must decrease with distance)");
  const int dim = c->dim;
  const int nx = c->P.mdim[0], ny = c->P.mdim[1], nz = dim == 3 ? c->P.mdim[2] : 1;
  const double res = c->P.res;
  const int rn = (int)std::ceil(radius[0] / res);
  const int hn = dim == 3 ? (int)std::ceil(radius[2] / res) : 0;
  if (rn < 1 || (dim == 3 && hn < 1)) return fail(MPLX_ERR_ARG, "potential radius smaller than one cell");
  const double h_max = 100;
  std::vector<double> avals;
  for (int i = 0; i <= rn; i++)
    for (int j = 0; j <= rn; j++)
      if (!(std::hypot(i, j) > rn)) avals.push_back(1 - (double)std::hypot(i, j) / rn);
  std::sort(avals.begin(), avals.end(), [](double a, double b) { return a > b; });
  avals.erase(std::unique(avals.begin(), avals.end()), avals.end());
  if (avals.size() >= (size_t)kNoRank) return fail(MPLX_ERR_ARG, "potential radius of %d cells is too large (rank table)", rn);
  std::vector<uint8_t> pair_rank((size_t)(rn + 1) * (rn + 1), (uint8_t)kNoRank);
  for (int i = 0; i <= rn; i++)
    for (int j = 0; j <= rn; j++) {
      if (std::hypot(i, j) > rn) continue;
      const double a = 1 - (double)std::hypot(i, j) / rn;
      const size_t rk = std::find(avals.begin(), avals.end(), a) - avals.begin();
      pair_rank[(size_t)j * (rn + 1) + i] = (uint8_t)rk;
    }
  std::vector<int8_t> htab(avals.size() * (hn + 1), (int8_t)-128);
  for (size_t rk = 0; rk < avals.size(); rk++)
    for (int z = 0; z <= hn; z++) {
      const double h = dim == 3 ? h_max * std::pow(avals[rk] * (1 - (double)z / hn), pow_) : h_max * std::pow(avals[rk], pow_);
      if (h > 1e-3) htab[rk * (hn + 1) + z] = (int8_t)h;
    }
  int lo[3] = {0, 0, 0}, hi[3] = {nx, ny, nz};
  double rnorm = 0;
  if (range)
    for (int k = 0; k < dim; k++) rnorm += range[k] * range[k];
  if (rnorm > 0) {
    if (!pos) return fail(MPLX_ERR_ARG, "pos is required with a potential map range");
    double a[3] = {0, 0, 0}, b[3] = {0, 0, 0};
    for (int k = 0; k < dim; k++) a[k] = pos[k] - range[k], b[k] = pos[k] + range[k];
    int c1[3], c2[3];
    float_to_int(c, a, c1);
    float_to_int(c, b, c2);
    for (int k = 0; k < dim; k++) {
      const int d = c->P.mdim[k];
      lo[k] = c1[k] < 0 ? 0 : (c1[k] >= d ? d - 1 : c1[k]);
      hi[k] = c2[k] < 0 ? 0 : (c2[k] >= d ? d - 1 : c2[k]);
    }
  }
  cudaStream_t st = c->stream;
  const size_t nvox = c->nvox;
  ScopedDevBuf<uint32_t> src;
  ScopedDevBuf<uint8_t> rank, d_pair;
  ScopedDevBuf<int8_t> d_htab;
  int rc = MPLX_OK;
  cudaError_t e = src.reserve((nvox + 31) / 32);
  if (e == cudaSuccess) e = rank.reserve(nvox);
  if (e == cudaSuccess) e = d_pair.reserve(pair_rank.size());
  if (e == cudaSuccess) e = d_htab.reserve(htab.size());
  if (e == cudaSuccess) e = c->pot.reserve(nvox);
  if (e == cudaSuccess) e = cudaMemcpyAsync(d_pair.p, pair_rank.data(), pair_rank.size(), cudaMemcpyHostToDevice, st);
  if (e == cudaSuccess) e = cudaMemcpyAsync(d_htab.p, htab.data(), htab.size(), cudaMemcpyHostToDevice, st);
  if (e == cudaSuccess) {
    source_bits_kernel<<<grid_for((nvox + 31) / 32), 256, 0, st>>>(c->map.p, nx, ny, nz, lo[0], lo[1], lo[2], hi[0], hi[1],
                                                                   hi[2], src.p);
    layer_rank_kernel<<<grid_for(nvox), 256, 0, st>>>(src.p, nx, ny, nz, rn, d_pair.p, rank.p);
    potential_combine_kernel<<<grid_for(nvox), 256, 0, st>>>(c->map.p, src.p, rank.p, nx, ny, nz, hn, d_htab.p, c->pot.p);
    e = cudaGetLastError();
    c->launches += 3;
  }
  if (e == cudaSuccess) e = cudaMemcpyAsync(c->map.p, c->pot.p, nvox, cudaMemcpyDeviceToDevice, st);
  if (e == cudaSuccess) e = launch_pack_bits(c->map.p, nvox, c->occ.p, true, st);
  if (e == cudaSuccess) e = launch_pack_occ2(c->occ.p, nvox, c->dim, nx, ny, nz, c->occ2.p, st);
  if (e == cudaSuccess && out_map) e = cudaMemcpyAsync(out_map, c->pot.p, nvox, cudaMemcpyDeviceToHost, st);
  if (e == cudaSuccess) e = cudaStreamSynchronize(st);
  src.release();
  rank.release();
  d_pair.release();
  d_htab.release();
  if (e != cudaSuccess) {
    cudaGetLastError();
    rc = fail(e == cudaErrorMemoryAllocation ? MPLX_ERR_ALLOC : MPLX_ERR_CUDA, "mplx_update_potential_map: %s",
              cudaGetErrorString(e));
    return rc;
  }
  c->launches++;
  c->has_pot = true;
  c->P.pot_w = potential_weight;
  c->P.grad_w = gradient_weight;
  c->P.pot = c->pot.p;
  return MPLX_OK;
}

search::Grid mplx::region_grid(const mplx_ctx *c) {
  search::Grid G{};
  G.map = nullptr;
  G.dim = c->dim;
  G.res = c->P.res;
  for (int k = 0; k < 3; k++) {
    G.mdim[k] = c->P.mdim[k];
    G.origin[k] = c->P.origin[k];
  }
  return G;
}

namespace {
struct PushCells {
  std::vector<int> *cells;
  void operator()(int, const int *pn) const { cells->insert(cells->end(), pn, pn + 3); }
};
}

static void region_path_cells(const mplx_ctx *c, const double *path, int n_pts, int dense, std::vector<int> &cells) {
  const int dim = c->dim;
  const search::Grid G = region_grid(c);
  const PushCells push{&cells};
  if (!dense) {
    for (int i = 1; i < n_pts; i++) search::segment_cells(G, path + (size_t)(i - 1) * dim, path + (size_t)i * dim, push);
  } else {
    for (int i = 0; i < n_pts; i++) {
      int pn[3] = {0, 0, 0};
      for (int k = 0; k < dim; k++) pn[k] = search::float_to_int(G, path[(size_t)i * dim + k], k);
      push(i, pn);
    }
  }
}

void mplx::region_radius_cells(const mplx_ctx *c, const double *radius, int *rn) {
  for (int k = 0; k < 3; k++) rn[k] = k < c->dim ? (int)std::ceil(radius[k] / c->P.res) : 0;
}

extern "C" int mplx_set_search_region_path(mplx_ctx *c, const double *path, int n_pts, const double *radius, int dense,
                                           uint8_t *out_region) {
  if (int r = mplx_bind(c)) return r;
  if (!c->has_map) return fail(MPLX_ERR_ARG, "mplx_set_map must be called first");
  if (!path || n_pts < 1 || !radius) return fail(MPLX_ERR_ARG, "path/radius missing");
  const int dim = c->dim;
  const int nx = c->P.mdim[0], ny = c->P.mdim[1], nz = dim == 3 ? c->P.mdim[2] : 1;
  std::vector<int> cells;
  region_path_cells(c, path, n_pts, dense, cells);
  int rn[3];
  region_radius_cells(c, radius, rn);
  cudaStream_t st = c->stream;
  const size_t nvox = c->nvox, nwords = (nvox + 31) / 32;
  const int ncell = (int)(cells.size() / 3);
  ScopedDevBuf<int> d_cells;
  CU(c->region.reserve(nwords));
  CU(cudaMemsetAsync(c->region.p, 0, nwords * sizeof(uint32_t), st));
  if (ncell > 0) {
    CU(d_cells.reserve(cells.size()));
    CU(cudaMemcpyAsync(d_cells.p, cells.data(), cells.size() * sizeof(int), cudaMemcpyHostToDevice, st));
    const size_t total = (size_t)ncell * (2 * rn[0] + 1) * (2 * rn[1] + 1) * (dim == 3 ? 2 * rn[2] + 1 : 1);
    region_stamp_kernel<<<grid_for(total), 256, 0, st>>>(d_cells.p, ncell, dim, nx, ny, nz, rn[0], rn[1], rn[2], c->region.p);
    CU(cudaGetLastError());
    c->launches++;
  }
  if (out_region) {
    std::vector<uint32_t> bits(nwords);
    CU(cudaMemcpyAsync(bits.data(), c->region.p, nwords * sizeof(uint32_t), cudaMemcpyDeviceToHost, st));
    CU(cudaStreamSynchronize(st));
    for (size_t i = 0; i < nvox; i++) out_region[i] = (bits[i >> 5] >> (i & 31)) & 1u;
  } else {
    CU(cudaStreamSynchronize(st));
  }
  d_cells.release();
  c->has_region = true;
  c->P.region_bits = c->region.p;
  return MPLX_OK;
}
```

### motion_primitive_library_b200/csrc/mplx_pack.cuh

```cuda
#pragma once
#include <stddef.h>
#include <stdint.h>

namespace mplx {

template <bool OCC>
__host__ __device__ inline uint32_t pack_word(const int8_t *bytes, size_t wd, size_t nvox) {
  uint32_t m = 0;
  const size_t b0 = wd << 5;
#pragma unroll 8
  for (int b = 0; b < 32; b++) {
    const size_t i = b0 + b;
    if (i < nvox && (OCC ? bytes[i] == 100 : bytes[i] != 0)) m |= 1u << b;
  }
  return m;
}

__host__ __device__ inline uint32_t range_bits(size_t wd, size_t lo, size_t hi) {
  const size_t b0 = wd << 5;
  const size_t a = lo > b0 ? lo - b0 : 0, c = hi < b0 + 32 ? (hi > b0 ? hi - b0 : 0) : 32;
  if (a >= c) return 0;
  return (c - a == 32 ? ~0u : ((1u << (c - a)) - 1u)) << a;
}

__host__ __device__ inline uint32_t occ_window(const uint32_t *occ, size_t nwords, long long s) {
  const long long w = s >> 5;
  const int r = (int)(s & 31);
  const uint32_t lo = w >= 0 && (size_t)w < nwords ? occ[w] : 0u;
  const uint32_t hi = w + 1 >= 0 && (size_t)(w + 1) < nwords ? occ[w + 1] : 0u;
  return r ? (lo >> r) | (hi << (32 - r)) : lo;
}

__host__ __device__ inline uint32_t occ2_summary_word(const uint32_t *occ, size_t wd, size_t nvox, int dim, int nx, int ny) {
  const size_t nwords = (nvox + 31) >> 5, sxy = (size_t)nx * ny, b0 = wd << 5;
  uint32_t d = range_bits(wd, nvox, ~(size_t)0);
  for (size_t i = b0 + (nx - b0 % nx) % nx; i < b0 + 32; i += nx) d |= 1u << (i - b0);
  for (size_t p = b0 / sxy; p * sxy < b0 + 32; p++) d |= range_bits(wd, p * sxy, p * sxy + nx);
  if (dim == 3) d |= range_bits(wd, 0, sxy);
  for (int dz = 0; dz <= (dim == 3 ? 1 : 0); dz++)
    for (int dy = 0; dy <= 1; dy++)
      for (int dx = 0; dx <= 1; dx++)
        d |= occ_window(occ, nwords, (long long)b0 - dx - (long long)dy * nx - (long long)dz * (long long)sxy);
  return d;
}

constexpr int kOcc2BrickPairs = 16;

__host__ __device__ inline int occ2_bricks_x(int dim, int nx) { return dim == 3 ? (nx + 7) >> 3 : (nx + 31) >> 5; }
__host__ __device__ inline int occ2_bricks_y(int dim, int ny) { return dim == 3 ? (ny + 7) >> 3 : (ny + 15) >> 4; }

__host__ __device__ inline size_t occ2_pair_count(int dim, int nx, int ny, int nz) {
  const size_t bz = dim == 3 ? (size_t)((nz + 7) >> 3) : 1;
  return (size_t)occ2_bricks_x(dim, nx) * occ2_bricks_y(dim, ny) * bz * kOcc2BrickPairs;
}

template <int DIM>
__host__ __device__ inline unsigned occ2_brick(int x, int y, int z, int nbx, int nby) {
  return DIM == 3 ? (unsigned)(x >> 3) + (unsigned)nbx * ((unsigned)(y >> 3) + (unsigned)nby * (unsigned)(z >> 3))
                  : (unsigned)(x >> 5) + (unsigned)nbx * (unsigned)(y >> 4);
}

template <int DIM>
__host__ __device__ inline unsigned occ2_pair(int x, int y, int z, int nbx, int nby) {
  const unsigned in_brick = DIM == 3 ? (unsigned)(((y >> 2) & 1) | ((z & 7) << 1)) : (unsigned)(y & 15);
  return occ2_brick<DIM>(x, y, z, nbx, nby) * kOcc2BrickPairs + in_brick;
}

template <int DIM>
__host__ __device__ inline unsigned occ2_bit(int x, int y) {
  return DIM == 3 ? (unsigned)((x & 7) | ((y & 3) << 3)) : (unsigned)(x & 31);
}

__host__ __device__ inline uint32_t occ2_summary_run(const uint32_t *occ, size_t s, int len, size_t nvox, int dim, int nx,
                                                     int ny) {
  const size_t w = s >> 5;
  const int r = (int)(s & 31);
  uint32_t v = occ2_summary_word(occ, w, nvox, dim, nx, ny) >> r;
  if (r + len > 32) v |= occ2_summary_word(occ, w + 1, nvox, dim, nx, ny) << (32 - r);
  return v;
}

__host__ __device__ inline void occ2_brick_pair(const uint32_t *occ, size_t p, size_t nvox, int dim, int nx, int ny, int nz,
                                                uint32_t &o, uint32_t &s) {
  const size_t nwords = (nvox + 31) >> 5;
  const size_t brick = p / kOcc2BrickPairs;
  const int q = (int)(p % kOcc2BrickPairs);
  const int nbx = occ2_bricks_x(dim, nx), nby = occ2_bricks_y(dim, ny);
  const int bx = (int)(brick % nbx);
  const size_t byz = brick / nbx;
  int x0, y0, z, run, rows;
  if (dim == 3) {
    x0 = bx * 8;
    y0 = (int)(byz % nby) * 8 + (q & 1) * 4;
    z = (int)(byz / nby) * 8 + (q >> 1);
    run = 8;
    rows = 4;
  } else {
    x0 = bx * 32;
    y0 = (int)byz * 16 + q;
    z = 0;
    run = 32;
    rows = 1;
  }
  o = s = ~0u;
  const int len = nx - x0 < run ? nx - x0 : run;
  const uint32_t m = len == 32 ? ~0u : (1u << len) - 1u;
  for (int r = 0; r < rows; r++) {
    const int y = y0 + r;
    if (y >= ny || z >= nz) continue;
    const size_t i = (size_t)x0 + (size_t)nx * ((size_t)y + (size_t)ny * z);
    const int sh = r * run;
    o = (o & ~(m << sh)) | ((occ_window(occ, nwords, (long long)i) & m) << sh);
    s = (s & ~(m << sh)) | ((occ2_summary_run(occ, i, len, nvox, dim, nx, ny) & m) << sh);
  }
}

}
```

### motion_primitive_library_b200/csrc/mplx_update.cu

```cuda
#include <cub/device/device_radix_sort.cuh>
#include <cuda_runtime.h>
#include <string.h>

#include "mplx_internal.h"
#include "mplx_pack.cuh"

namespace mplx {

__global__ void scatter_last_kernel(const uint32_t *__restrict__ idx, const int8_t *__restrict__ val, int n,
                                    int8_t *__restrict__ map) {
  for (int k = blockIdx.x * blockDim.x + threadIdx.x; k < n; k += gridDim.x * blockDim.x)
    if (k == n - 1 || idx[k + 1] != idx[k]) map[idx[k]] = val[k];
}

__device__ __forceinline__ bool first_of_word(const uint32_t *idx, int k) {
  return k == 0 || (idx[k - 1] >> 5) != (idx[k] >> 5);
}

__global__ void repack_occ_kernel(const uint32_t *__restrict__ idx, int n, const int8_t *__restrict__ map, size_t nvox,
                                  uint32_t *__restrict__ occ) {
  for (int k = blockIdx.x * blockDim.x + threadIdx.x; k < n; k += gridDim.x * blockDim.x)
    if (first_of_word(idx, k)) occ[idx[k] >> 5] = pack_word<true>(map, idx[k] >> 5, nvox);
}

__global__ void repack_occ2_kernel(const uint32_t *__restrict__ idx, int n, const uint32_t *__restrict__ occ, size_t nvox,
                                   int dim, int nx, int ny, int nz, uint32_t *__restrict__ occ2) {
  const size_t npairs = occ2_pair_count(dim, nx, ny, nz);
  const size_t sxy = (size_t)nx * ny;
  const int nbx = occ2_bricks_x(dim, nx), nby = occ2_bricks_y(dim, ny);
  const int xmask = dim == 3 ? 7 : 31;
  for (int k = blockIdx.x * blockDim.x + threadIdx.x; k < n; k += gridDim.x * blockDim.x) {
    const uint32_t v = idx[k];
    const int x = (int)(v % nx), y = (int)(v / nx % ny), z = (int)(v / sxy);
    if (k > 0 && (idx[k - 1] == v || (idx[k - 1] == v - 1 && (x & xmask) != 0 && (x & xmask) != xmask))) continue;
    unsigned done[8];
    int nd = 0;
    for (int dz = 0; dz <= (dim == 3 ? 1 : 0); dz++)
      for (int dy = 0; dy <= 1; dy++)
        for (int dx = 0; dx <= 1; dx++) {
          if (x + dx >= nx || y + dy >= ny || z + dz >= nz) continue;
          const unsigned p = dim == 3 ? occ2_pair<3>(x + dx, y + dy, z + dz, nbx, nby)
                                      : occ2_pair<2>(x + dx, y + dy, 0, nbx, nby);
          bool seen = false;
          for (int i = 0; i < nd; i++) seen = seen || done[i] == p;
          if (seen) continue;
          done[nd++] = p;
          uint32_t o, s;
          occ2_brick_pair(occ, p, nvox, dim, nx, ny, nz, o, s);
          occ2[p] = o;
          occ2[npairs + p] = s;
        }
  }
}

__global__ void unbrick_occ2_kernel(const uint32_t *__restrict__ occ2, size_t npairs, size_t nvox, int dim, int nx,
                                    int ny, uint2 *__restrict__ out) {
  const size_t nwords = (nvox + 31) >> 5, sxy = (size_t)nx * ny;
  const int nbx = occ2_bricks_x(dim, nx), nby = occ2_bricks_y(dim, ny);
  for (size_t w = (size_t)blockIdx.x * blockDim.x + threadIdx.x; w < nwords; w += (size_t)gridDim.x * blockDim.x) {
    uint32_t o = 0, s = 0;
    for (int b = 0; b < 32; b++) {
      const size_t i = (w << 5) + b;
      if (i >= nvox) {
        s |= 1u << b;
        continue;
      }
      const int x = (int)(i % nx), y = (int)(i / nx % ny), z = (int)(i / sxy);
      const unsigned p = dim == 3 ? occ2_pair<3>(x, y, z, nbx, nby) : occ2_pair<2>(x, y, 0, nbx, nby);
      const unsigned bit = dim == 3 ? occ2_bit<3>(x, y) : occ2_bit<2>(x, y);
      o |= ((occ2[p] >> bit) & 1u) << b;
      s |= ((occ2[npairs + p] >> bit) & 1u) << b;
    }
    out[w] = make_uint2(o, s);
  }
}

static int grid_for_entries(int n) {
  const int cap = sm_count() * 16;
  const int g = (n + 255) / 256;
  return g < 1 ? 1 : (g > cap ? cap : g);
}

}

using namespace mplx;

extern "C" int mplx_update_cells(mplx_ctx *c, const int32_t *idx, const int8_t *values, int n) {
  if (int r = mplx_bind(c)) return r;
  if (!c->has_map) return fail(MPLX_ERR_ARG, "mplx_set_map must be called first");
  if (n < 0) return fail(MPLX_ERR_ARG, "n = %d < 0", n);
  if (n == 0) return MPLX_OK;
  if (!idx || !values) return fail(MPLX_ERR_ARG, "idx/values is null");
  bool sorted = true;
  for (int k = 0; k < n; k++) {
    if (idx[k] < 0 || (size_t)idx[k] >= c->nvox)
      return fail(MPLX_ERR_ARG, "idx[%d] = %d is outside the grid [0, %zu)", k, idx[k], c->nvox);
    sorted = sorted && (k == 0 || idx[k] >= idx[k - 1]);
  }
  UpdateBufs &B = c->ub;
  cudaStream_t st = c->stream;
  CU(B.h_idx.reserve(n));
  CU(B.h_val.reserve(n));
  CU(B.idx.reserve(n));
  CU(B.val.reserve(n));
  memcpy(B.h_idx.p, idx, sizeof(int32_t) * n);
  memcpy(B.h_val.p, values, n);
  CU(cudaMemcpyAsync(B.idx.p, B.h_idx.p, sizeof(uint32_t) * n, cudaMemcpyHostToDevice, st));
  CU(cudaMemcpyAsync(B.val.p, B.h_val.p, n, cudaMemcpyHostToDevice, st));
  const uint32_t *d_idx = B.idx.p;
  const int8_t *d_val = B.val.p;
  if (!sorted) {
    int end_bit = 1;
    while (end_bit < 32 && ((c->nvox - 1) >> end_bit) != 0) end_bit++;
    CU(B.idx_sorted.reserve(n));
    CU(B.val_sorted.reserve(n));
    size_t tmp_bytes = 0;
    CU(cub::DeviceRadixSort::SortPairs(nullptr, tmp_bytes, B.idx.p, B.idx_sorted.p, B.val.p, B.val_sorted.p, n, 0, end_bit,
                                       st));
    CU(B.sort_tmp.reserve(tmp_bytes));
    CU(cub::DeviceRadixSort::SortPairs(B.sort_tmp.p, tmp_bytes, B.idx.p, B.idx_sorted.p, B.val.p, B.val_sorted.p, n, 0,
                                       end_bit, st));
    d_idx = B.idx_sorted.p;
    d_val = B.val_sorted.p;
  }
  const int grid = grid_for_entries(n);
  const int nx = c->P.mdim[0], ny = c->P.mdim[1], nz = c->dim == 3 ? c->P.mdim[2] : 1;
  scatter_last_kernel<<<grid, 256, 0, st>>>(d_idx, d_val, n, c->map.p);
  repack_occ_kernel<<<grid, 256, 0, st>>>(d_idx, n, c->map.p, c->nvox, c->occ.p);
  repack_occ2_kernel<<<grid, 256, 0, st>>>(d_idx, n, c->occ.p, c->nvox, c->dim, nx, ny, nz, c->occ2.p);
  CU(cudaGetLastError());
  c->launches += 3;
  CU(cudaStreamSynchronize(st));
  return MPLX_OK;
}

extern "C" int mplx_read_map(mplx_ctx *c, int8_t *grid, uint32_t *occ, uint32_t *occ2) {
  if (int r = mplx_bind(c)) return r;
  if (!c->has_map) return fail(MPLX_ERR_ARG, "mplx_set_map must be called first");
  const size_t nwords = (c->nvox + 31) / 32;
  cudaStream_t st = c->stream;
  if (grid) CU(cudaMemcpyAsync(grid, c->map.p, c->nvox, cudaMemcpyDeviceToHost, st));
  if (occ) CU(cudaMemcpyAsync(occ, c->occ.p, nwords * sizeof(uint32_t), cudaMemcpyDeviceToHost, st));
  if (occ2) {
    ScopedDevBuf<uint2> tmp;
    CU(tmp.reserve(nwords));
    const int grid = grid_for_entries(nwords < (1u << 30) ? (int)nwords : 1 << 30);
    unbrick_occ2_kernel<<<grid, 256, 0, st>>>(c->occ2.p, c->P.occ2_sum, c->nvox, c->dim, c->P.mdim[0], c->P.mdim[1],
                                              tmp.p);
    CU(cudaGetLastError());
    c->launches += 1;
    CU(cudaMemcpyAsync(occ2, tmp.p, nwords * sizeof(uint2), cudaMemcpyDeviceToHost, st));
    CU(cudaStreamSynchronize(st));
  }
  CU(cudaStreamSynchronize(st));
  return MPLX_OK;
}
```

Baseline: 386.2 million.

## Pad occ2 brick map with guard band and drop per-sample bounds checks

Rebuilds the bricked two-level occupancy map with a guard margin of occupied bricks around the grid and computes brick word indices through a separable affine formula on the raw double high words. A per-primitive band test, based on a Bernstein-style bound of the polynomial reach, proves a trajectory stays inside the guard so the inner sampling loop can skip per-sample inside checks and masking. The L2 persistence window sizing moves into a helper that is rerun on every parameter refresh. The trade-offs are a larger occ2 footprint, an extra per-primitive bound computation, and a new CHECK template variant that falls back to the checked path when the guard is too small or a region mask is set.

```diff
diff --git a/motion_primitive_library_b200/csrc/mplx_api.cu b/motion_primitive_library_b200/csrc/mplx_api.cu
--- a/motion_primitive_library_b200/csrc/mplx_api.cu
+++ b/motion_primitive_library_b200/csrc/mplx_api.cu
@@ -30,6 +30,26 @@
   return MPLX_OK;
 }
 
+void mplx::size_l2_window(mplx_ctx *c) {
+  size_t bytes = 0;
+  int maxp = 0, maxw = 0;
+  if (c->has_map && !c->has_pot && (c->P.control & 16) == 0 && c->P.occ2_sum <= (1u << 27)) {
+    cudaDeviceGetAttribute(&maxp, cudaDevAttrMaxPersistingL2CacheSize, c->device);
+    cudaDeviceGetAttribute(&maxw, cudaDevAttrMaxAccessPolicyWindowSize, c->device);
+    const size_t half = (size_t)c->P.occ2_sum * sizeof(uint32_t);
+    if (maxp > 0 && maxw > 0) bytes = 2 * half <= (size_t)maxp ? 2 * half : half;
+  }
+  const size_t want = bytes < (size_t)maxp ? bytes : (size_t)maxp;
+  if (want != c->l2_persist) {
+    if (cudaDeviceSetLimit(cudaLimitPersistingL2CacheSize, want) != cudaSuccess) {
+      cudaGetLastError();
+      bytes = 0;
+    }
+    c->l2_persist = want;
+  }
+  c->occ2_window = bytes < (size_t)maxw ? bytes : (size_t)maxw;
+}
+
 static void refresh_params(mplx_ctx *c) {
   c->P.map = c->has_map ? c->map.p : nullptr;
   c->P.pot = c->has_pot ? c->pot.p : nullptr;
@@ -38,6 +58,7 @@
   c->P.stats = c->stats_on ? c->stats.p : nullptr;
   c->P.occ_bits = c->has_map ? c->occ.p : nullptr;
   c->P.occ2 = c->has_map ? c->occ2.p : nullptr;
+  mplx::size_l2_window(c);
   c->P.occ2_bytes = c->has_map ? c->occ2_window : 0;
   c->P.prow = c->prow.p;
   c->P.row_u = c->row_u.p;
@@ -136,25 +157,10 @@
   CU(c->occ.reserve((nvox + 31) / 32));
   CU(mplx::launch_pack_bits(c->map.p, nvox, c->occ.p, true, c->stream));
   const int nz = c->dim == 3 ? dim[2] : 1;
-  const size_t npairs = mplx::occ2_pair_count(c->dim, dim[0], dim[1], nz);
+  const size_t npairs = mplx::occ2_guard_pair_count(c->dim, dim[0], dim[1], nz);
   CU(c->occ2.reserve(2 * npairs));
   CU(mplx::launch_pack_occ2(c->occ.p, nvox, c->dim, dim[0], dim[1], nz, c->occ2.p, c->stream));
   c->launches += 2;
-  {
-    int maxp = 0, maxw = 0;
-    cudaDeviceGetAttribute(&maxp, cudaDevAttrMaxPersistingL2CacheSize, c->device);
-    cudaDeviceGetAttribute(&maxw, cudaDevAttrMaxAccessPolicyWindowSize, c->device);
-    const size_t half = npairs * sizeof(uint32_t);
-    const size_t bytes = 2 * half <= (size_t)maxp ? 2 * half : half;
-    c->occ2_window = 0;
-    if (maxp > 0 && maxw > 0) {
-      const size_t want = bytes < (size_t)maxp ? bytes : (size_t)maxp;
-      if (cudaDeviceSetLimit(cudaLimitPersistingL2CacheSize, want) == cudaSuccess)
-        c->occ2_window = bytes < (size_t)maxw ? bytes : (size_t)maxw;
-      else
-        cudaGetLastError();
-    }
-  }
   CU(cudaStreamSynchronize(c->stream));
   c->nvox = nvox;
   for (int k = 0; k < 3; k++) {
@@ -162,9 +168,8 @@
     c->P.origin[k] = k < c->dim ? origin[k] : 0.0;
     c->P.dimd[k] = (double)c->P.mdim[k];
   }
-  c->P.occ2_nb[0] = mplx::occ2_bricks_x(c->dim, dim[0]);
-  c->P.occ2_nb[1] = mplx::occ2_bricks_y(c->dim, dim[1]);
-  c->P.occ2_sum = (unsigned)npairs;
+  mplx::occ2_sep_terms(c->dim, dim[0], dim[1], mplx::kFxHiBase, c->P.occ2_e, c->P.occ2_k0);
+  c->P.occ2_sum = npairs < ((size_t)1 << 32) ? (unsigned)npairs : ~0u;
   c->P.res = res;
   c->P.rinv = 1.0 / res;
   c->has_map = true;
diff --git a/motion_primitive_library_b200/csrc/mplx_device.cuh b/motion_primitive_library_b200/csrc/mplx_device.cuh
--- a/motion_primitive_library_b200/csrc/mplx_device.cuh
+++ b/motion_primitive_library_b200/csrc/mplx_device.cuh
@@ -28,12 +28,15 @@
   const uint32_t *occ2;
   unsigned occ2_sum;
   size_t occ2_bytes;
-  int occ2_nb[2];
+  unsigned occ2_e[3], occ2_k0;
   const unsigned char *prow;
   const double *row_u;
   const unsigned char *row_axis;
   int n_rows;
 };
+
+constexpr double kFxMagic = 1572864.0;
+constexpr int kFxHiBase = 0x41380000;
 
 constexpr int kNMax = 128;
 constexpr int kTStride = kNMax + 2;
diff --git a/motion_primitive_library_b200/csrc/mplx_fx.cu b/motion_primitive_library_b200/csrc/mplx_fx.cu
--- a/motion_primitive_library_b200/csrc/mplx_fx.cu
+++ b/motion_primitive_library_b200/csrc/mplx_fx.cu
@@ -60,7 +60,7 @@
   }
 }
 
-template <int DIM, int ORD, int UNR, int MINB, bool LAT, bool REGION>
+template <int DIM, int ORD, int UNR, int MINB, bool LAT, bool REGION, bool CHECK>
 __global__ void __launch_bounds__(kFxThreads, MINB)
 expand_fx_kernel(const __grid_constant__ EnvParams P, const mplx_waypoint *__restrict__ nodes, int n_nodes, int npb,
                  int inv_nU, const __grid_constant__ OutPtrs o) {
@@ -184,15 +184,19 @@
       double reach = 0.0;
 #pragma unroll
       for (int a = 0; a < DIM; a++) reach = fmax(reach, (fabs(pr.ax[a].c5) + fabs(P.origin[a])) * P.rinv);
-      if (n > kNMax || !(reach < kFxRange)) {
+      double C[DIM][ORD + 1];
+      bool band = true;
+#pragma unroll
+      for (int a = 0; a < DIM; a++) {
+        fx_axis<ORD>(pr.ax[a], P.origin[a], P.rinv, C[a]);
+        if (!REGION && !CHECK) band = band && fx_band<ORD>(C[a], P.T, P.mdim[a]);
+      }
+      if (n > kNMax || !(reach < kFxRange) || !band) {
         double cf[CoefLayout<DIM, ORD, false>::NCMAX];
         fill_coef<DIM, ORD, false>(pr, false, cf);
         unsigned ns = 0;
         verdict = isinf(traverse_loop<DIM, ORD, false>(P, cf, false, max_v, ns)) ? 1 : 0;
       } else {
-        double C[DIM][ORD + 1];
-#pragma unroll
-        for (int a = 0; a < DIM; a++) fx_axis<ORD>(pr.ax[a], P.origin[a], P.rinv, C[a]);
         const unsigned *__restrict__ occ_words = P.occ2;
         unsigned long long amask = 0;
         bool full = false;
@@ -200,7 +204,7 @@
         int base = 0;
         for (int left = __ldg(P.tcount + n);; left -= UNR, base += UNR) {
           unsigned amb;
-          const int st = fx_group<DIM, ORD, UNR, REGION>(P, occ_words, C, dt, left, t, amb);
+          const int st = fx_group<DIM, ORD, UNR, REGION, CHECK>(P, occ_words, C, dt, left, t, amb);
           if (st == 2) {
             verdict = 1;
             break;
@@ -231,7 +235,8 @@
 }
 
 bool fx_supported(const EnvParams &P) {
-  return P.occ2 != nullptr && P.pot == nullptr && (P.control & 16) == 0 && P.nU <= kThreads && P.stats == nullptr;
+  return P.occ2 != nullptr && P.occ2_sum <= (1u << 27) && P.pot == nullptr && (P.control & 16) == 0 && P.nU <= kThreads &&
+         P.stats == nullptr;
 }
 
 cudaError_t launch_expand_fx(const EnvParams &P, const mplx_waypoint *d_nodes, int n_nodes, const OutPtrs &o,
@@ -252,17 +257,20 @@
     return with_order(P.control, [&](auto ORD) {
       return with_bool(unr == 8, [&](auto UNR8) {
         return with_bool(o.lattice != nullptr, [&](auto LAT) {
-          return with_bool(P.region_bits != nullptr, [&](auto REGION) {
-            auto launch = [&](auto MINB) {
-              expand_fx_kernel<DIM, ORD, UNR8 ? 8 : 4, MINB, LAT, REGION>
+          return with_bool(P.region_bits != nullptr || P.maxn + 2 > kOcc2Guard, [&](auto CHECK) {
+            auto launch = [&](auto MINB, auto REGION) {
+              expand_fx_kernel<DIM, ORD, UNR8 ? 8 : 4, MINB, LAT, REGION, CHECK>
                   <<<grid, kFxThreads, 0, st>>>(P, d_nodes, n_nodes, npb, inv_nU, o);
               return cudaGetLastError();
             };
-            if constexpr (DIM == 3 && ORD == 2 && !LAT && !REGION) {
-              if (minb_env == 5) return launch(Int<5>());
-              if (minb_env == 6) return launch(Int<6>());
+            if constexpr (CHECK) {
+              if (P.region_bits != nullptr) return launch(Int<4>(), std::true_type{});
             }
-            return launch(Int<4>());
+            if constexpr (DIM == 3 && ORD == 2 && !LAT) {
+              if (minb_env == 5) return launch(Int<5>(), std::false_type{});
+              if (minb_env == 6) return launch(Int<6>(), std::false_type{});
+            }
+            return launch(Int<4>(), std::false_type{});
           });
         });
       });
@@ -272,10 +280,10 @@
 
 __global__ void pack_occ2_kernel(const uint32_t *__restrict__ occ, size_t nvox, int dim, int nx, int ny, int nz,
                                  uint32_t *__restrict__ out) {
-  const size_t npairs = occ2_pair_count(dim, nx, ny, nz);
+  const size_t npairs = occ2_guard_pair_count(dim, nx, ny, nz);
   for (size_t p = (size_t)blockIdx.x * blockDim.x + threadIdx.x; p < npairs; p += (size_t)gridDim.x * blockDim.x) {
     uint32_t o, s;
-    occ2_brick_pair(occ, p, nvox, dim, nx, ny, nz, o, s);
+    occ2_guard_brick_pair(occ, p, nvox, dim, nx, ny, nz, o, s);
     out[p] = o;
     out[npairs + p] = s;
   }
@@ -283,7 +291,7 @@
 
 cudaError_t launch_pack_occ2(const uint32_t *d_occ, size_t nvox, int dim, int nx, int ny, int nz, uint32_t *d_out,
                              cudaStream_t st) {
-  const size_t npairs = occ2_pair_count(dim, nx, ny, nz);
+  const size_t npairs = occ2_guard_pair_count(dim, nx, ny, nz);
   int grid = (int)((npairs + 255) / 256);
   if (grid > sm_count() * 16) grid = sm_count() * 16;
   if (grid < 1) grid = 1;
diff --git a/motion_primitive_library_b200/csrc/mplx_fx.cuh b/motion_primitive_library_b200/csrc/mplx_fx.cuh
--- a/motion_primitive_library_b200/csrc/mplx_fx.cuh
+++ b/motion_primitive_library_b200/csrc/mplx_fx.cuh
@@ -4,8 +4,6 @@
 
 namespace mplx {
 
-constexpr double kFxMagic = 1572864.0;
-constexpr int kFxHiBase = 0x41380000;
 constexpr double kFxEps = 0x1p-26;
 constexpr unsigned kFxUnc = 128u;
 constexpr double kFxRange = 131072.0;
@@ -23,20 +21,32 @@
   C[0] = (q[0] - origin) * rinv + (kFxMagic + kFxEps);
 }
 
+template <int ORD>
+__device__ __forceinline__ bool fx_band(const double (&C)[ORD + 1], double T, int mdim) {
+  if ((unsigned)(__double2hiint(C[0]) - kFxHiBase) >= (unsigned)mdim) return false;
+  return occ2_band_reach<ORD>(C, T) + 2.0 <= (double)kOcc2Guard;
+}
+
 __device__ __forceinline__ unsigned rotr_wrap(unsigned x, unsigned s) {
   unsigned r;
   asm("shf.r.wrap.b32 %0, %1, %1, %2;" : "=r"(r) : "r"(x), "r"(s));
   return r;
 }
 
-template <int DIM, int ORD, int UNR, bool REGION>
-__device__ __forceinline__ int fx_group(const EnvParams &P, const unsigned *__restrict__ base,
-                                        const double (&C)[DIM][ORD + 1], double dt, int left, double &t, unsigned &amb) {
+template <int UNR>
+struct FxWords {
   unsigned w[UNR], rot[UNR];
-  unsigned uncm = 0;
+  unsigned uncm;
+};
+
+template <int DIM, int ORD, int UNR, bool REGION, bool CHECK>
+__device__ __forceinline__ void fx_issue(const EnvParams &P, const unsigned *__restrict__ base,
+                                         const double (&C)[DIM][ORD + 1], double dt, int left, double &t,
+                                         FxWords<UNR> &G) {
+  G.uncm = 0;
 #pragma unroll
   for (int j = 0; j < UNR; j++) {
-    int cell[DIM];
+    int hi[DIM];
     unsigned lo[DIM];
     bool inside = true;
 #pragma unroll
@@ -45,110 +55,73 @@
 #pragma unroll
       for (int i = ORD - 1; i >= 1; i--) h = __fma_rn(h, t, C[a][i]);
       const double m = __fma_rn(h, t, C[a][0]);
-      cell[a] = __double2hiint(m) - kFxHiBase;
+      hi[a] = __double2hiint(m);
       lo[a] = (unsigned)__double2loint(m);
-      inside = inside && ((unsigned)cell[a] < (unsigned)P.mdim[a]);
-    }
-    const unsigned fr = DIM == 3 ? min(min(lo[0], lo[1]), lo[DIM - 1]) : min(lo[0], lo[1]);
-    const unsigned ub = fr < kFxUnc ? 1u : 0u;
-    uncm += ub << j;
-    w[j] = 0xffffffffu;
-    if (REGION) {
-      int idx = cell[0] + P.mdim[0] * cell[1];
-      if (DIM == 3) idx += P.mdim[0] * P.mdim[1] * cell[DIM - 1];
-      rot[j] = (unsigned)(idx - j);
-      if (inside && !ub) {
-        const unsigned wi = (unsigned)idx >> 5;
-        w[j] = __ldg(P.occ_bits + wi) | ~__ldg(P.region_bits + wi);
-      }
-    } else {
-      const int z = DIM == 3 ? cell[DIM - 1] : 0;
-      rot[j] = occ2_bit<DIM>(cell[0], cell[1]) - j;
-      if (inside) w[j] = __ldg(base + (occ2_pair<DIM>(cell[0], cell[1], z, P.occ2_nb[0], P.occ2_nb[1]) + (ub ? P.occ2_sum : 0u)));
-    }
-    t += dt;
-  }
-  unsigned r = 0;
-#pragma unroll
-  for (int j = 0; j < UNR; j++) r |= rotr_wrap(w[j], rot[j]) & (1u << j);
-  if (left < UNR) r &= (1u << left) - 1u;
-  amb = r & uncm;
-  if (r & ~uncm) return 2;
-  return left <= UNR ? 1 : 0;
-}
-
-template <int UNR>
-struct FxWords {
-  unsigned w[UNR], rot[UNR];
-  unsigned uncm;
-};
-
-template <int DIM, int ORD, int UNR, bool REGION>
-__device__ __forceinline__ void fx_issue(const EnvParams &P, const unsigned *__restrict__ base,
-                                         const double (&C)[DIM][ORD + 1], double dt, double &t, FxWords<UNR> &G) {
-  G.uncm = 0;
-#pragma unroll
-  for (int j = 0; j < UNR; j++) {
-    int cell[DIM];
-    unsigned lo[DIM];
-    bool inside = true;
-#pragma unroll
-    for (int a = 0; a < DIM; a++) {
-      double h = C[a][ORD];
-#pragma unroll
-      for (int i = ORD - 1; i >= 1; i--) h = __fma_rn(h, t, C[a][i]);
-      const double m = __fma_rn(h, t, C[a][0]);
-      cell[a] = __double2hiint(m) - kFxHiBase;
-      lo[a] = (unsigned)__double2loint(m);
-      inside = inside && ((unsigned)cell[a] < (unsigned)P.mdim[a]);
+      if (REGION || CHECK) inside = inside && ((unsigned)(hi[a] - kFxHiBase) < (unsigned)P.mdim[a]);
     }
     const unsigned fr = DIM == 3 ? min(min(lo[0], lo[1]), lo[DIM - 1]) : min(lo[0], lo[1]);
     const unsigned ub = fr < kFxUnc ? 1u : 0u;
     G.uncm += ub << j;
-    G.w[j] = 0xffffffffu;
     if (REGION) {
-      int idx = cell[0] + P.mdim[0] * cell[1];
-      if (DIM == 3) idx += P.mdim[0] * P.mdim[1] * cell[DIM - 1];
+      int idx = (hi[0] - kFxHiBase) + P.mdim[0] * (hi[1] - kFxHiBase);
+      if (DIM == 3) idx += P.mdim[0] * P.mdim[1] * (hi[DIM - 1] - kFxHiBase);
       G.rot[j] = (unsigned)(idx - j);
+      G.w[j] = 0xffffffffu;
       if (inside && !ub) {
         const unsigned wi = (unsigned)idx >> 5;
         G.w[j] = __ldg(P.occ_bits + wi) | ~__ldg(P.region_bits + wi);
       }
     } else {
-      const int z = DIM == 3 ? cell[DIM - 1] : 0;
-      G.rot[j] = occ2_bit<DIM>(cell[0], cell[1]) - j;
-      if (inside) G.w[j] = __ldg(base + (occ2_pair<DIM>(cell[0], cell[1], z, P.occ2_nb[0], P.occ2_nb[1]) + (ub ? P.occ2_sum : 0u)));
+      const unsigned k = occ2_sep_k<DIM>(hi, P.occ2_e, P.occ2_k0);
+      G.rot[j] = k - j;
+      const unsigned *wp = base + ((k >> 5) + (ub ? P.occ2_sum : 0u));
+      if (CHECK) {
+        G.w[j] = 0xffffffffu;
+        if (inside) G.w[j] = __ldg(wp);
+      } else {
+        G.w[j] = 0u;
+        if (j == 0 || j < left) G.w[j] = __ldg(wp);
+      }
     }
     t += dt;
   }
 }
 
-template <int UNR>
+template <int UNR, bool MASK>
 __device__ __forceinline__ int fx_decide(const FxWords<UNR> &G, int left, unsigned &amb) {
   unsigned r = 0;
 #pragma unroll
   for (int j = 0; j < UNR; j++) r |= rotr_wrap(G.w[j], G.rot[j]) & (1u << j);
-  if (left < UNR) r &= (1u << left) - 1u;
+  if (MASK && left < UNR) r &= (1u << left) - 1u;
   amb = r & G.uncm;
   if (r & ~G.uncm) return 2;
   return left <= UNR ? 1 : 0;
 }
 
-template <int DIM, int ORD, int UNR, bool REGION>
+template <int DIM, int ORD, int UNR, bool REGION, bool CHECK>
+__device__ __forceinline__ int fx_group(const EnvParams &P, const unsigned *__restrict__ base,
+                                        const double (&C)[DIM][ORD + 1], double dt, int left, double &t, unsigned &amb) {
+  FxWords<UNR> G;
+  fx_issue<DIM, ORD, UNR, REGION, CHECK>(P, base, C, dt, left, t, G);
+  return fx_decide<UNR, REGION || CHECK>(G, left, amb);
+}
+
+template <int DIM, int ORD, int UNR, bool REGION, bool CHECK>
 __device__ __forceinline__ int fx_traverse(const EnvParams &P, const double (&C)[DIM][ORD + 1], double dt, int count,
                                            unsigned long long &amask, bool &full) {
+  constexpr bool MASK = REGION || CHECK;
   const unsigned *__restrict__ base = P.occ2;
   amask = 0;
   full = false;
   double t = 0;
   int left = count, k0 = 0;
   FxWords<UNR> A, B;
-  fx_issue<DIM, ORD, UNR, REGION>(P, base, C, dt, t, A);
+  fx_issue<DIM, ORD, UNR, REGION, CHECK>(P, base, C, dt, left, t, A);
   for (;;) {
     unsigned amb;
     int st;
-    if (left > UNR) fx_issue<DIM, ORD, UNR, REGION>(P, base, C, dt, t, B);
-    st = fx_decide<UNR>(A, left, amb);
+    if (left > UNR) fx_issue<DIM, ORD, UNR, REGION, CHECK>(P, base, C, dt, left - UNR, t, B);
+    st = fx_decide<UNR, MASK>(A, left, amb);
     if (st == 2) return 1;
     if (amb) {
       if (k0 + UNR <= 64) amask |= (unsigned long long)amb << k0; else full = true;
@@ -156,8 +129,8 @@
     if (st == 1) return 0;
     left -= UNR;
     k0 += UNR;
-    if (left > UNR) fx_issue<DIM, ORD, UNR, REGION>(P, base, C, dt, t, A);
-    st = fx_decide<UNR>(B, left, amb);
+    if (left > UNR) fx_issue<DIM, ORD, UNR, REGION, CHECK>(P, base, C, dt, left - UNR, t, A);
+    st = fx_decide<UNR, MASK>(B, left, amb);
     if (st == 2) return 1;
     if (amb) {
       if (k0 + UNR <= 64) amask |= (unsigned long long)amb << k0; else full = true;
diff --git a/motion_primitive_library_b200/csrc/mplx_fxn.cu b/motion_primitive_library_b200/csrc/mplx_fxn.cu
--- a/motion_primitive_library_b200/csrc/mplx_fxn.cu
+++ b/motion_primitive_library_b200/csrc/mplx_fxn.cu
@@ -16,7 +16,7 @@
   uint64_t km[ORD];
   unsigned char f0, f1, f2, pad[5];
 };
-constexpr unsigned char kSame = 1, kReach = 2, kVel = 1, kAcc = 1, kJrk = 2;
+constexpr unsigned char kSame = 1, kReach = 2, kVel = 1, kAcc = 1, kJrk = 2, kBand = 4;
 
 
 struct FxnWork {
@@ -60,7 +60,7 @@
   if (c.tail) bulk_copy(d + at, s + at, c.tail);
 }
 
-template <int DIM, int ORD, int UNR, int MINB, bool LAT, bool REGION, bool SORT, bool STAGE>
+template <int DIM, int ORD, int UNR, int MINB, bool LAT, bool REGION, bool CHECK, bool SORT, bool STAGE>
 __global__ void __launch_bounds__(kThreads, MINB)
 expand_fxn_kernel(const __grid_constant__ EnvParams P, const mplx_waypoint *__restrict__ nodes, int n_nodes, int npb,
                   int inv_nU, int inv_rows, FxAmbRec *__restrict__ amb_q, unsigned *__restrict__ amb_n,
@@ -148,6 +148,7 @@
         if (ORD >= 3) Rw.km[ORD >= 3 ? 2 : 0] = hash_premix(Rw.id[2]);
         if (ORD >= 4) Rw.km[ORD >= 4 ? 3 : 0] = hash_premix(Rw.id[3]);
         unsigned char f = kAcc | kJrk;
+        if (!REGION && !CHECK && fx_band<ORD>(Rw.C, T, a == 0 ? P.mdim[0] : (a == 1 ? P.mdim[1] : P.mdim[2]))) f |= kBand;
         if (ORD >= 3 && P.a_max > 0 && ax.max_acc(T) > P.a_max) f &= ~kAcc;
         if (ORD >= 4 && P.j_max > 0 && ax.max_jrk(T) > P.j_max) f &= ~kJrk;
         Rw.f2 = f;
@@ -187,14 +188,14 @@
   const int ci = item - nl * nU;
   const int ni = node0 + nl;
   const bool active = item < items && ni < n_nodes;
-  bool ok = false, same = true, reach = true;
+  bool ok = false, same = true, reach = true, band = true;
   double max_v = 0;
   uint64_t key = 0;
   int ra[DIM];
 #pragma unroll
   for (int a = 0; a < DIM; a++) ra[a] = 0;
   if (active) {
-    unsigned f0 = kSame | kReach, f1 = kVel, f2 = kAcc | kJrk;
+    unsigned f0 = kSame | kReach, f1 = kVel, f2 = kAcc | kJrk | kBand;
 #pragma unroll
     for (int a = 0; a < DIM; a++) {
       ra[a] = nl * n_rows + __ldg(P.prow + ci * 3 + a);
@@ -204,9 +205,10 @@
       f2 &= Rw.f2;
       if (Rw.mv > max_v) max_v = Rw.mv;
     }
-    ok = f1 == kVel && f2 == (kAcc | kJrk);
+    ok = f1 == kVel && (f2 & (kAcc | kJrk)) == (kAcc | kJrk);
     same = (f0 & kSame) != 0;
     reach = (f0 & kReach) != 0;
+    band = (f2 & kBand) != 0;
     if (ok) {
 #pragma unroll
       for (int a = 0; a < DIM; a++) {
@@ -220,7 +222,7 @@
 
   int n = 0, count = 0;
   double dt = 0.0;
-  const bool literal = emit && !same && !reach;
+  const bool literal = emit && !same && !(reach && (REGION || CHECK || band));
   bool beyond = false;
   if (emit && !same) {
     n = sample_count_n(P, max_v, dt);
@@ -422,7 +424,7 @@
 #pragma unroll
     for (int a = 1; a < DIM; a++) J += rows[wr[a]].J;
     wintr = J + P.w * P.T;
-    verdict = fx_traverse<DIM, ORD, UNR, REGION>(P, C, __ldg(P.tdt + wn), __ldg(P.tcount + wn), amask, full);
+    verdict = fx_traverse<DIM, ORD, UNR, REGION, CHECK>(P, C, __ldg(P.tdt + wn), __ldg(P.tcount + wn), amask, full);
     if (verdict == 0 && (amask != 0 || full)) verdict = 2;
   }
   const unsigned am = __ballot_sync(0xffffffffu, verdict == 2);
@@ -592,9 +594,9 @@
       }
       if ((mask & 4) && sg.succ >= 0 && o.cost && smem + span_slots * 8 + 32 + sizeof(FxnShared) <= kCtaSmem)
         sg.cost = take(span_slots * 8);
-      auto launch = [&](auto UNR, auto MINB, auto LAT, auto REGION) {
+      auto launch = [&](auto UNR, auto MINB, auto LAT, auto REGION, auto CHECK) {
         auto go = [&](auto SORT, auto STAGE) {
-          const auto kernel = expand_fxn_kernel<DIM, ORD, UNR, MINB, LAT, REGION, SORT, STAGE>;
+          const auto kernel = expand_fxn_kernel<DIM, ORD, UNR, MINB, LAT, REGION, CHECK, SORT, STAGE>;
           if (smem > 32 * 1024) {
             const cudaError_t r = cudaFuncSetAttribute(kernel, cudaFuncAttributeMaxDynamicSharedMemorySize, (int)smem);
             if (r != cudaSuccess) return r;
@@ -612,13 +614,15 @@
       };
       const std::true_type yes{};
       const std::false_type no{};
-      if (region) e = with_bool(lat, [&](auto LAT) { return launch(Int<4>(), Int<4>(), LAT, yes); });
-      else if (lat) e = launch(Int<4>(), Int<4>(), yes, no);
-      else if (unr_env == 8 && minb_env == 3) e = launch(Int<8>(), Int<3>(), no, no);
-      else if (unr_env == 4 && minb_env == 3) e = launch(Int<4>(), Int<3>(), no, no);
-      else if (unr_env == 8) e = launch(Int<8>(), Int<4>(), no, no);
-      else if (minb_env == 5) e = launch(Int<4>(), Int<5>(), no, no);
-      else e = launch(Int<4>(), Int<4>(), no, no);
+      const bool check = P.maxn + 2 > kOcc2Guard;
+      if (region) e = with_bool(lat, [&](auto LAT) { return launch(Int<4>(), Int<4>(), LAT, yes, yes); });
+      else if (lat) e = with_bool(check, [&](auto CHECK) { return launch(Int<4>(), Int<4>(), yes, no, CHECK); });
+      else if (check) e = launch(Int<4>(), Int<4>(), no, no, yes);
+      else if (unr_env == 8 && minb_env == 3) e = launch(Int<8>(), Int<3>(), no, no, no);
+      else if (unr_env == 4 && minb_env == 3) e = launch(Int<4>(), Int<3>(), no, no, no);
+      else if (unr_env == 8) e = launch(Int<8>(), Int<4>(), no, no, no);
+      else if (minb_env == 5) e = launch(Int<4>(), Int<5>(), no, no, no);
+      else e = launch(Int<4>(), Int<4>(), no, no, no);
       if (e != cudaSuccess) return e;
       return with_bool(region, [&](auto REGION) {
         fx_resolve_kernel<DIM, ORD, REGION><<<kFxSegments * 8, 128, 0, st>>>(P, d_nodes, q, amb_n, amb_cap, o.cost);
diff --git a/motion_primitive_library_b200/csrc/mplx_internal.h b/motion_primitive_library_b200/csrc/mplx_internal.h
--- a/motion_primitive_library_b200/csrc/mplx_internal.h
+++ b/motion_primitive_library_b200/csrc/mplx_internal.h
@@ -265,6 +265,7 @@
   DevBuf<double> row_u;
   int n_rows = 0;
   size_t occ2_window = 0;
+  size_t l2_persist = 0;
   DevBuf<double> U, ttab, tdt;
   DevBuf<int> tcount;
   int kernel = 0;
@@ -297,6 +298,7 @@
 struct Grid;
 }
 search::Grid region_grid(const mplx_ctx *c);
+void size_l2_window(mplx_ctx *c);
 void region_radius_cells(const mplx_ctx *c, const double *radius, int *rn);
 int search_budget(const mplx_ctx *c, size_t &budget);
 }
diff --git a/motion_primitive_library_b200/csrc/mplx_maps.cu b/motion_primitive_library_b200/csrc/mplx_maps.cu
--- a/motion_primitive_library_b200/csrc/mplx_maps.cu
+++ b/motion_primitive_library_b200/csrc/mplx_maps.cu
@@ -201,6 +201,8 @@
   c->P.pot_w = potential_weight;
   c->P.grad_w = gradient_weight;
   c->P.pot = c->pot.p;
+  size_l2_window(c);
+  c->P.occ2_bytes = c->occ2_window;
   return MPLX_OK;
 }
 
diff --git a/motion_primitive_library_b200/csrc/mplx_pack.cuh b/motion_primitive_library_b200/csrc/mplx_pack.cuh
--- a/motion_primitive_library_b200/csrc/mplx_pack.cuh
+++ b/motion_primitive_library_b200/csrc/mplx_pack.cuh
@@ -1,4 +1,5 @@
 #pragma once
+#include <math.h>
 #include <stddef.h>
 #include <stdint.h>
 
@@ -45,6 +46,7 @@
 }
 
 constexpr int kOcc2BrickPairs = 16;
+constexpr int kOcc2Guard = 32;
 
 __host__ __device__ inline int occ2_bricks_x(int dim, int nx) { return dim == 3 ? (nx + 7) >> 3 : (nx + 31) >> 5; }
 __host__ __device__ inline int occ2_bricks_y(int dim, int ny) { return dim == 3 ? (ny + 7) >> 3 : (ny + 15) >> 4; }
@@ -80,39 +82,122 @@
   return v;
 }
 
+__host__ __device__ inline void occ2_pair_words(const uint32_t *occ, int bx0, int by0, int bz0, int q, size_t nvox,
+                                                int dim, int nx, int ny, int nz, uint32_t &o, uint32_t &s) {
+  const size_t nwords = (nvox + 31) >> 5;
+  int y0, z, run, rows;
+  if (dim == 3) {
+    y0 = by0 + (q & 1) * 4;
+    z = bz0 + (q >> 1);
+    run = 8;
+    rows = 4;
+  } else {
+    y0 = by0 + q;
+    z = 0;
+    run = 32;
+    rows = 1;
+  }
+  o = s = ~0u;
+  if (bx0 < 0 || bx0 >= nx || z < 0 || z >= nz) return;
+  const int len = nx - bx0 < run ? nx - bx0 : run;
+  const uint32_t m = len == 32 ? ~0u : (1u << len) - 1u;
+  for (int r = 0; r < rows; r++) {
+    const int y = y0 + r;
+    if (y < 0 || y >= ny) continue;
+    const size_t i = (size_t)bx0 + (size_t)nx * ((size_t)y + (size_t)ny * z);
+    const int sh = r * run;
+    o = (o & ~(m << sh)) | ((occ_window(occ, nwords, (long long)i) & m) << sh);
+    s = (s & ~(m << sh)) | ((occ2_summary_run(occ, i, len, nvox, dim, nx, ny) & m) << sh);
+  }
+}
+
 __host__ __device__ inline void occ2_brick_pair(const uint32_t *occ, size_t p, size_t nvox, int dim, int nx, int ny, int nz,
                                                 uint32_t &o, uint32_t &s) {
-  const size_t nwords = (nvox + 31) >> 5;
   const size_t brick = p / kOcc2BrickPairs;
-  const int q = (int)(p % kOcc2BrickPairs);
   const int nbx = occ2_bricks_x(dim, nx), nby = occ2_bricks_y(dim, ny);
   const int bx = (int)(brick % nbx);
   const size_t byz = brick / nbx;
-  int x0, y0, z, run, rows;
-  if (dim == 3) {
-    x0 = bx * 8;
-    y0 = (int)(byz % nby) * 8 + (q & 1) * 4;
-    z = (int)(byz / nby) * 8 + (q >> 1);
-    run = 8;
-    rows = 4;
-  } else {
-    x0 = bx * 32;
-    y0 = (int)byz * 16 + q;
-    z = 0;
-    run = 32;
-    rows = 1;
-  }
-  o = s = ~0u;
-  const int len = nx - x0 < run ? nx - x0 : run;
-  const uint32_t m = len == 32 ? ~0u : (1u << len) - 1u;
-  for (int r = 0; r < rows; r++) {
-    const int y = y0 + r;
-    if (y >= ny || z >= nz) continue;
-    const size_t i = (size_t)x0 + (size_t)nx * ((size_t)y + (size_t)ny * z);
-    const int sh = r * run;
-    o = (o & ~(m << sh)) | ((occ_window(occ, nwords, (long long)i) & m) << sh);
-    s = (s & ~(m << sh)) | ((occ2_summary_run(occ, i, len, nvox, dim, nx, ny) & m) << sh);
-  }
-}
-
-}
+  const int q = (int)(p % kOcc2BrickPairs);
+  if (dim == 3)
+    occ2_pair_words(occ, bx * 8, (int)(byz % nby) * 8, (int)(byz / nby) * 8, q, nvox, dim, nx, ny, nz, o, s);
+  else
+    occ2_pair_words(occ, bx * 32, (int)byz * 16, 0, q, nvox, dim, nx, ny, nz, o, s);
+}
+
+__host__ __device__ inline int occ2_guard_bricks_x(int dim, int nx) { return occ2_bricks_x(dim, nx + 2 * kOcc2Guard); }
+__host__ __device__ inline int occ2_guard_bricks_y(int dim, int ny) { return occ2_bricks_y(dim, ny + 2 * kOcc2Guard); }
+__host__ __device__ inline int occ2_guard_bricks_z(int dim, int nz) { return dim == 3 ? (nz + 2 * kOcc2Guard + 7) >> 3 : 1; }
+__host__ __device__ inline size_t occ2_guard_pair_count(int dim, int nx, int ny, int nz) {
+  return (size_t)occ2_guard_bricks_x(dim, nx) * occ2_guard_bricks_y(dim, ny) * occ2_guard_bricks_z(dim, nz) * kOcc2BrickPairs;
+}
+
+template <int DIM>
+__host__ __device__ inline unsigned occ2_guard_pair(int x, int y, int z, int pbx, int pby) {
+  return occ2_pair<DIM>(x + kOcc2Guard, y + kOcc2Guard, DIM == 3 ? z + kOcc2Guard : 0, pbx, pby);
+}
+
+__host__ __device__ inline void occ2_guard_brick_pair(const uint32_t *occ, size_t p, size_t nvox, int dim, int nx, int ny,
+                                                      int nz, uint32_t &o, uint32_t &s) {
+  const size_t brick = p / kOcc2BrickPairs;
+  const int pbx = occ2_guard_bricks_x(dim, nx), pby = occ2_guard_bricks_y(dim, ny);
+  const int bx = (int)(brick % pbx);
+  const size_t byz = brick / pbx;
+  const int q = (int)(p % kOcc2BrickPairs), G = kOcc2Guard;
+  if (dim == 3)
+    occ2_pair_words(occ, bx * 8 - G, (int)(byz % pby) * 8 - G, (int)(byz / pby) * 8 - G, q, nvox, dim, nx, ny, nz, o, s);
+  else
+    occ2_pair_words(occ, bx * 32 - G, (int)byz * 16 - G, 0, q, nvox, dim, nx, ny, nz, o, s);
+}
+
+template <int DIM>
+__host__ __device__ constexpr unsigned occ2_sep_scale(int a) { return DIM == 3 ? 1u << (3 * a) : (a == 0 ? 1u : 32u); }
+template <int DIM>
+__host__ __device__ constexpr int occ2_sep_shift(int a) { return DIM == 3 ? 3 : (a == 0 ? 5 : 4); }
+
+template <int DIM>
+__host__ __device__ inline unsigned occ2_sep_k(const int (&h)[DIM], const unsigned (&e)[3], unsigned k0) {
+  unsigned k = k0;
+#pragma unroll
+  for (int a = 0; a < DIM; a++) k += occ2_sep_scale<DIM>(a) * (unsigned)h[a] + (unsigned)(h[a] >> occ2_sep_shift<DIM>(a)) * e[a];
+  return k;
+}
+
+template <int ORD>
+__host__ __device__ inline double occ2_band_reach(const double (&C)[ORD + 1], double T) {
+  double a[ORD + 1], p = T;
+  for (int i = 1; i <= ORD; i++) {
+    a[i] = C[i] * p;
+    p *= T;
+  }
+  double m = 0.0;
+  for (int k = 1; k <= ORD; k++) {
+    double b = 0.0, ck = 1.0, cn = 1.0;
+    for (int i = 1; i <= k; i++) {
+      ck = ck * (k - i + 1) / i;
+      cn = cn * (ORD - i + 1) / i;
+      b += ck / cn * a[i];
+    }
+    m = fmax(m, fabs(b));
+  }
+  return m;
+}
+
+template <int DIM>
+inline void occ2_sep_terms_dim(int pbx, int pby, int H, unsigned (&e)[3], unsigned &k0) {
+  const unsigned D[3] = {512u, 512u * (unsigned)pbx, 512u * (unsigned)pbx * (unsigned)pby};
+  const int B = H - kOcc2Guard;
+  k0 = 0;
+  e[0] = e[1] = e[2] = 0;
+  for (int a = 0; a < DIM; a++) {
+    e[a] = D[a] - (occ2_sep_scale<DIM>(a) << occ2_sep_shift<DIM>(a));
+    k0 -= occ2_sep_scale<DIM>(a) * (unsigned)B + (unsigned)(B >> occ2_sep_shift<DIM>(a)) * e[a];
+  }
+}
+
+inline void occ2_sep_terms(int dim, int nx, int ny, int H, unsigned (&e)[3], unsigned &k0) {
+  const int pbx = occ2_guard_bricks_x(dim, nx), pby = occ2_guard_bricks_y(dim, ny);
+  if (dim == 3) occ2_sep_terms_dim<3>(pbx, pby, H, e, k0);
+  else occ2_sep_terms_dim<2>(pbx, pby, H, e, k0);
+}
+
+}
diff --git a/motion_primitive_library_b200/csrc/mplx_update.cu b/motion_primitive_library_b200/csrc/mplx_update.cu
--- a/motion_primitive_library_b200/csrc/mplx_update.cu
+++ b/motion_primitive_library_b200/csrc/mplx_update.cu
@@ -25,9 +25,9 @@
 
 __global__ void repack_occ2_kernel(const uint32_t *__restrict__ idx, int n, const uint32_t *__restrict__ occ, size_t nvox,
                                    int dim, int nx, int ny, int nz, uint32_t *__restrict__ occ2) {
-  const size_t npairs = occ2_pair_count(dim, nx, ny, nz);
+  const size_t npairs = occ2_guard_pair_count(dim, nx, ny, nz);
   const size_t sxy = (size_t)nx * ny;
-  const int nbx = occ2_bricks_x(dim, nx), nby = occ2_bricks_y(dim, ny);
+  const int pbx = occ2_guard_bricks_x(dim, nx), pby = occ2_guard_bricks_y(dim, ny);
   const int xmask = dim == 3 ? 7 : 31;
   for (int k = blockIdx.x * blockDim.x + threadIdx.x; k < n; k += gridDim.x * blockDim.x) {
     const uint32_t v = idx[k];
@@ -39,14 +39,14 @@
       for (int dy = 0; dy <= 1; dy++)
         for (int dx = 0; dx <= 1; dx++) {
           if (x + dx >= nx || y + dy >= ny || z + dz >= nz) continue;
-          const unsigned p = dim == 3 ? occ2_pair<3>(x + dx, y + dy, z + dz, nbx, nby)
-                                      : occ2_pair<2>(x + dx, y + dy, 0, nbx, nby);
+          const unsigned p = dim == 3 ? occ2_guard_pair<3>(x + dx, y + dy, z + dz, pbx, pby)
+                                      : occ2_guard_pair<2>(x + dx, y + dy, 0, pbx, pby);
           bool seen = false;
           for (int i = 0; i < nd; i++) seen = seen || done[i] == p;
           if (seen) continue;
           done[nd++] = p;
           uint32_t o, s;
-          occ2_brick_pair(occ, p, nvox, dim, nx, ny, nz, o, s);
+          occ2_guard_brick_pair(occ, p, nvox, dim, nx, ny, nz, o, s);
           occ2[p] = o;
           occ2[npairs + p] = s;
         }
@@ -56,7 +56,7 @@
 __global__ void unbrick_occ2_kernel(const uint32_t *__restrict__ occ2, size_t npairs, size_t nvox, int dim, int nx,
                                     int ny, uint2 *__restrict__ out) {
   const size_t nwords = (nvox + 31) >> 5, sxy = (size_t)nx * ny;
-  const int nbx = occ2_bricks_x(dim, nx), nby = occ2_bricks_y(dim, ny);
+  const int pbx = occ2_guard_bricks_x(dim, nx), pby = occ2_guard_bricks_y(dim, ny);
   for (size_t w = (size_t)blockIdx.x * blockDim.x + threadIdx.x; w < nwords; w += (size_t)gridDim.x * blockDim.x) {
     uint32_t o = 0, s = 0;
     for (int b = 0; b < 32; b++) {
@@ -66,7 +66,7 @@
         continue;
       }
       const int x = (int)(i % nx), y = (int)(i / nx % ny), z = (int)(i / sxy);
-      const unsigned p = dim == 3 ? occ2_pair<3>(x, y, z, nbx, nby) : occ2_pair<2>(x, y, 0, nbx, nby);
+      const unsigned p = dim == 3 ? occ2_guard_pair<3>(x, y, z, pbx, pby) : occ2_guard_pair<2>(x, y, 0, pbx, pby);
       const unsigned bit = dim == 3 ? occ2_bit<3>(x, y) : occ2_bit<2>(x, y);
       o |= ((occ2[p] >> bit) & 1u) << b;
       s |= ((occ2[npairs + p] >> bit) & 1u) << b;
@@ -145,8 +145,8 @@
     ScopedDevBuf<uint2> tmp;
     CU(tmp.reserve(nwords));
     const int grid = grid_for_entries(nwords < (1u << 30) ? (int)nwords : 1 << 30);
-    unbrick_occ2_kernel<<<grid, 256, 0, st>>>(c->occ2.p, c->P.occ2_sum, c->nvox, c->dim, c->P.mdim[0], c->P.mdim[1],
-                                              tmp.p);
+    const size_t npairs = occ2_guard_pair_count(c->dim, c->P.mdim[0], c->P.mdim[1], c->dim == 3 ? c->P.mdim[2] : 1);
+    unbrick_occ2_kernel<<<grid, 256, 0, st>>>(c->occ2.p, npairs, c->nvox, c->dim, c->P.mdim[0], c->P.mdim[1], tmp.p);
     CU(cudaGetLastError());
     c->launches += 1;
     CU(cudaMemcpyAsync(occ2, tmp.p, nwords * sizeof(uint2), cudaMemcpyDeviceToHost, st));
```

Measured after the change: 434.7 million, median of 6. 1.13x the previous value.
